# DomhnallBoyle/lip2speech-unit

Hardware: AMD Instinct MI355X
Metric: real-time factor (audio-sec/wall-sec), end-to-end lip->16kHz audio, 4s@25fps clips (higher is better)
Workload: dtype fp16

## Files before the change

include/lip2speech_hip.h:

```cpp
#ifndef LIP2SPEECH_HIP_H
#define LIP2SPEECH_HIP_H

#include <stddef.h>
#include <stdint.h>

#ifdef __cplusplus
extern "C" {
#endif

#define L2S_ABI_VERSION 16

enum { L2S_F16 = 0, L2S_BF16 = 1, L2S_F32 = 2 };

enum { L2S_OK = 0, L2S_EINVAL = -1, L2S_ESHAPE = -2, L2S_EALIGN = -3, L2S_EUNSUPPORTED = -4 };

enum {
  L2S_ACT_NONE = 0,
  L2S_ACT_RELU = 1,
  L2S_ACT_GELU = 2,
  L2S_ACT_SWISH = 3,
  L2S_ACT_PRELU = 4,
  L2S_ACT_LRELU = 5,
  L2S_ACT_TANH = 6
};

enum {
  L2S_F_RES_PRE  = 1 << 0,
  L2S_F_RES_POST = 1 << 1,
  L2S_F_ACCUM    = 1 << 2,
  L2S_F_DUAL     = 1 << 3,
  L2S_F_MASK     = 1 << 4,
  L2S_F_OUT_F32  = 1 << 5,
  L2S_F_RES_F32  = 1 << 6
};

enum {
  L2S_MODE_LINEAR = 0,
  L2S_MODE_CONV1D = 1,
  L2S_MODE_CONV2D = 2
};

typedef struct l2s_gemm_desc {
  const void* A;
  const void* W;
  void* C;
  void* C2;
  const float* bias;
  const float* slope;
  const void* R;
  const int32_t* lens;
  int32_t M, N, Cin, ntaps;
  int32_t lda, ldc, ldc2, ldr;
  int32_t mode;
  int32_t T_out, T_in, stride, dil, off;
  int32_t Ho, Wo, Hi, Wi, KW, pad;
  int32_t out_row_mul, out_row_add;
  int32_t mask_T, mask_mul;
  int32_t act, flags, dtype;
  float alpha;
  float act_slope;
  float slope2;
  int32_t groups, a_gstride, c_gstride;
  int64_t w_gstride;
  const int32_t* ktab;
} l2s_gemm_desc;
#define L2S_KTAB_MAX 9

int l2s_abi_version(void);
const char* l2s_build_info(void);

int l2s_tapgemm(const l2s_gemm_desc* host_desc, void* stream);
#define L2S_VARIANT_F32 2128128
int l2s_tapgemm_variant(const l2s_gemm_desc* host_desc);
#define L2S_EPI_FAMILY_F32 32
int l2s_tapgemm_epilogue_family(const l2s_gemm_desc* host_desc);

int l2s_stem_conv3d(const void* x, int x_is_f32, const void* w, const float* bias, const float* slope,
                    void* y, int B, int T, int H, int W, int dtype, void* stream);

int l2s_stem_pool_fused(const void* x, int x_is_f32, const void* w, const float* bias, const float* slope,
                        void* y, int B, int T, int H, int W, int dtype, void* stream);

int l2s_stem_pool_fused_u8(const uint8_t* frames, int Hin, int Win, int crop, float mean, float std, const void* w,
                           const float* bias, const float* slope, void* y, int B, int T, int dtype, void* stream);

int l2s_maxpool2d_3x3s2(const void* x, void* y, int N, int H, int W, int C, int dtype, void* stream);

int l2s_avgpool_hw(const void* x, void* y, int N, int HW, int C, int dtype, void* stream);

int l2s_layernorm(const void* x, int x_is_f32, int ldx, const float* gamma, const float* beta, float eps,
                  void* y, int y_is_f32, int ldy, void* y2, int ldy2, int M, int C, int zero_prefix,
                  const int32_t* lens, int len_mul, int mask_T, int dtype, void* stream);

int l2s_attention(const void* qkv, int ldq, void* out, int ldo, const void* pos, int ldp,
                  const float* bias_u, const float* bias_v, const int32_t* lens, int len_mul,
                  int B, int T, int H, int dtype, void* stream);

int l2s_glu_dwconv_swish(const void* x, const float* w, const float* bias, void* y, const int32_t* lens,
                         int len_mul, int B, int T, int C, int k, int dtype, void* stream);

int l2s_greedy_decode(const float* logits, int ldl, const int32_t* lens, int len_mul, int B, int T2, int V,
                      float temperature, float lenpen, int32_t* tokens, float* lprobs, float* score, void* stream);

int l2s_beam_decode(const float* logits, int ldl, const int32_t* lens, int len_mul, int B, int T2, int V, float temperature,
                    float lenpen, int beam, void* workspace, size_t workspace_bytes, int32_t* tokens, float* pos_scores,
                    float* score, int32_t* nhyp, void* stream);
size_t l2s_beam_decode_workspace(int B, int T2, int beam);

int l2s_ctc_frames(const float* logits, int ldl, const int32_t* lens, int len_mul, int B, int L, int V, int K, int32_t* labels,
                   int32_t* topk_cls, float* topk_lp, void* stream);

int l2s_ctc_beam_search(const int32_t* topk_cls, const float* topk_lp, const int32_t* lens, int len_mul, int B, int L, int K,
                        int beam, int nbest, void* workspace, size_t workspace_bytes, int32_t* labels, int32_t* lengths,
                        float* scores, void* stream);
size_t l2s_ctc_beam_workspace(int B, int L, int beam);
int l2s_ctc_repeat_labels(const int32_t* x, int ldx, const int32_t* lens, int len_mul, int B, int L, int32_t* y, int ldy,
                          void* stream);

int l2s_repeat2_cast(const float* x, void* y, int B, int T, int C, int dtype, void* stream);

int l2s_splitk_reduce(const float* P, int ldp, int S, float* x, int ldx, int M, int N, void* stream);

int l2s_splitk_reduce_layernorm(const float* P, int ldp, int S, float* x, int ldx, const float* gamma, const float* beta, float eps,
                                void* y, int y_is_f32, int ldy, int M, int C, const int32_t* lens, int len_mul, int mask_T,
                                int dtype, void* stream);

int l2s_cast_f32_to_16(const float* x, int ldx, void* y, int ldy, int M, int C, int dtype, void* stream);
int l2s_cast_16_to_f32(const void* x, int ldx, float* y, int ldy, int M, int C, int dtype, void* stream);
int l2s_broadcast_rows(const void* v, int ldv, void* y, int ldy, int col0, const int32_t* lens, int len_mul,
                       int B, int T, int C, int v_is_f32, int dtype, void* stream);
int l2s_transpose_ct_to_tc(const float* x, void* y, int ldy, int col0, const int32_t* lens, int len_mul,
                           int B, int C, int T, int dtype, void* stream);
int l2s_embedding(const int32_t* code, const void* table, void* y, int ldy, const int32_t* lens,
                  int B, int L, int C, int dtype, void* stream);
int l2s_embedding_tokens(const int32_t* tok, int ldt, int token_offset, const void* table, int n_rows, void* y, int ldy,
                         const int32_t* lens, int len_mul, int B, int L, int C, int dtype, void* stream);
int l2s_rows_f32_to_16_masked(const float* x, int ldx, void* y, int ldy, int col0, const int32_t* lens, int len_mul,
                              int B, int T, int C, int dtype, void* stream);
int l2s_lens_from_mask(const uint8_t* mask, int32_t* lens, int B, int T, void* stream);
int l2s_split_hi_lo(const float* x, int ldx, void* hi, void* lo, int ld16, int act, float slope, const int32_t* lens,
                    int len_mul, int B, int T, int C, int dtype, void* stream);

typedef struct l2s_respair_desc {
  const void* X; const void* W1; const void* W2; const float* b1; const float* b2;
  void* Y; float* XS; const int32_t* lens;
  int32_t len_mul, B, T, C, k, dil, last, accumulate, dtype;
  float slope;
} l2s_respair_desc;
int l2s_respair(const l2s_respair_desc* d, void* stream);

typedef struct l2s_respair_final_desc {
  const void* X[3]; const void* W1[3]; const void* W2[3]; const float* b1[3]; const float* b2[3];
  int32_t k[3], dil[3];
  void* Y; const int32_t* lens;
  int32_t n, len_mul, B, T, C, dtype;
  float slope;
} l2s_respair_final_desc;
int l2s_respair_final(const l2s_respair_final_desc* d, void* stream);

int l2s_basicblock_fused(const void* x, const void* w1, const float* b1, const float* s1, const void* w2, const float* b2,
                         const float* s2, void* y, int n_images, int H, int W, int C, int dtype, void* stream);
int l2s_basiclayer_fused(const void* x, const void* const* w, const float* const* bias, const float* const* slope, int n_blocks,
                         void* y, int n_images, int H, int W, int C, int dtype, void* stream);
int l2s_basicstage128_tail_fused(const void* x0, const void* t0, const void* wa, const float* ba, const float* sa, const void* w1,
                                 const float* b1, const float* s1, const void* w2, const float* b2, const float* s2, void* y,
                                 int n_images, int H, int W, int dtype, void* stream);

int l2s_conv_post_tanh(const float* x, const float* w, float bias, float* wav, int16_t* pcm, const int32_t* lens,
                       int len_mul, int B, int T, int C, int k, void* stream);

int l2s_resblock_fused(const void* xl, const void* w, const float* bias, float* xs, void* xl_out,
                       const int32_t* lens, int len_mul, int B, int T, int C, int k, int d0, int d1, int d2,
                       int accumulate, float slope, int dtype, void* stream);

int l2s_resstage_fused(const void* xl, const void* const* w, const float* const* bias, const int* ks, const int* dils,
                       int n_blocks, float* xs, void* xl_out, const int32_t* lens, int len_mul, int B, int T, int C,
                       float slope, int xs_final, int dtype, void* stream);

int l2s_preprocess_frames(const uint8_t* frames, void* y, int B, int T, int Hin, int Win, int crop, float mean,
                          float std, int dtype, void* stream);

int l2s_mel_spectrogram(const void* wav, int wav_is_i16, int64_t ldw, const int32_t* n_samples, int B, int S, const float* basis,
                        const float* fb, const int32_t* fb_range, float* mel, int ldm, int T_rows, int n_fft, int hop,
// ... 43 lines not shown
```

lip2speech_unit_amd/_lib.py:

```python
import ctypes
import os

_HERE = os.path.dirname(os.path.abspath(__file__))
LIB_PATH = os.environ.get("L2S_LIB_PATH") or os.path.join(_HERE, "liblip2speech_hip.so")

F16, BF16, F32 = 0, 1, 2
ACT_NONE, ACT_RELU, ACT_GELU, ACT_SWISH, ACT_PRELU, ACT_LRELU, ACT_TANH = range(7)
F_RES_PRE, F_RES_POST, F_ACCUM, F_DUAL, F_MASK, F_OUT_F32, F_RES_F32 = (1 << i for i in range(7))
MODE_LINEAR, MODE_CONV1D, MODE_CONV2D = 0, 1, 2
ABI_VERSION = 16

_ERR = {-1: "L2S_EINVAL", -2: "L2S_ESHAPE", -3: "L2S_EALIGN", -4: "L2S_EUNSUPPORTED"}


class L2SError(RuntimeError):
    pass


class GemmDesc(ctypes.Structure):
    _fields_ = [
        ("A", ctypes.c_void_p), ("W", ctypes.c_void_p), ("C", ctypes.c_void_p), ("C2", ctypes.c_void_p),
        ("bias", ctypes.c_void_p), ("slope", ctypes.c_void_p), ("R", ctypes.c_void_p), ("lens", ctypes.c_void_p),
        ("M", ctypes.c_int32), ("N", ctypes.c_int32), ("Cin", ctypes.c_int32), ("ntaps", ctypes.c_int32),
        ("lda", ctypes.c_int32), ("ldc", ctypes.c_int32), ("ldc2", ctypes.c_int32), ("ldr", ctypes.c_int32),
        ("mode", ctypes.c_int32),
        ("T_out", ctypes.c_int32), ("T_in", ctypes.c_int32), ("stride", ctypes.c_int32), ("dil", ctypes.c_int32),
        ("off", ctypes.c_int32),
        ("Ho", ctypes.c_int32), ("Wo", ctypes.c_int32), ("Hi", ctypes.c_int32), ("Wi", ctypes.c_int32),
        ("KW", ctypes.c_int32), ("pad", ctypes.c_int32),
        ("out_row_mul", ctypes.c_int32), ("out_row_add", ctypes.c_int32),
        ("mask_T", ctypes.c_int32), ("mask_mul", ctypes.c_int32),
        ("act", ctypes.c_int32), ("flags", ctypes.c_int32), ("dtype", ctypes.c_int32),
        ("alpha", ctypes.c_float), ("act_slope", ctypes.c_float), ("slope2", ctypes.c_float),
        ("groups", ctypes.c_int32), ("a_gstride", ctypes.c_int32), ("c_gstride", ctypes.c_int32),
        ("w_gstride", ctypes.c_int64),
        ("ktab", ctypes.c_void_p),
    ]


_vp, _i, _f = ctypes.c_void_p, ctypes.c_int, ctypes.c_float


class RespairDesc(ctypes.Structure):
    _fields_ = [("X", ctypes.c_void_p), ("W1", ctypes.c_void_p), ("W2", ctypes.c_void_p), ("b1", ctypes.c_void_p),
                ("b2", ctypes.c_void_p), ("Y", ctypes.c_void_p), ("XS", ctypes.c_void_p), ("lens", ctypes.c_void_p),
                ("len_mul", ctypes.c_int32), ("B", ctypes.c_int32), ("T", ctypes.c_int32), ("C", ctypes.c_int32),
                ("k", ctypes.c_int32), ("dil", ctypes.c_int32), ("last", ctypes.c_int32), ("accumulate", ctypes.c_int32),
                ("dtype", ctypes.c_int32), ("slope", ctypes.c_float)]


class RespairFinalDesc(ctypes.Structure):
    _fields_ = [("X", ctypes.c_void_p * 3), ("W1", ctypes.c_void_p * 3), ("W2", ctypes.c_void_p * 3), ("b1", ctypes.c_void_p * 3),
                ("b2", ctypes.c_void_p * 3), ("k", ctypes.c_int32 * 3), ("dil", ctypes.c_int32 * 3),
                ("Y", ctypes.c_void_p), ("lens", ctypes.c_void_p),
                ("n", ctypes.c_int32), ("len_mul", ctypes.c_int32), ("B", ctypes.c_int32), ("T", ctypes.c_int32),
                ("C", ctypes.c_int32), ("dtype", ctypes.c_int32), ("slope", ctypes.c_float)]


SIGNATURES = {
    "l2s_abi_version": ([], ctypes.c_int),
    "l2s_build_info": ([], ctypes.c_char_p),
    "l2s_tapgemm": ([ctypes.POINTER(GemmDesc), _vp], _i),
    "l2s_tapgemm_variant": ([ctypes.POINTER(GemmDesc)], _i),
    "l2s_tapgemm_epilogue_family": ([ctypes.POINTER(GemmDesc)], _i),
    "l2s_stem_conv3d": ([_vp, _i, _vp, _vp, _vp, _vp, _i, _i, _i, _i, _i, _vp], _i),
    "l2s_stem_pool_fused": ([_vp, _i, _vp, _vp, _vp, _vp, _i, _i, _i, _i, _i, _vp], _i),
    "l2s_stem_pool_fused_u8": ([_vp, _i, _i, _i, _f, _f, _vp, _vp, _vp, _vp, _i, _i, _i, _vp], _i),
    "l2s_maxpool2d_3x3s2": ([_vp, _vp, _i, _i, _i, _i, _i, _vp], _i),
    "l2s_avgpool_hw": ([_vp, _vp, _i, _i, _i, _i, _vp], _i),
    "l2s_layernorm": ([_vp, _i, _i, _vp, _vp, _f, _vp, _i, _i, _vp, _i, _i, _i, _i, _vp, _i, _i, _i, _vp], _i),
    "l2s_attention": ([_vp, _i, _vp, _i, _vp, _i, _vp, _vp, _vp, _i, _i, _i, _i, _i, _vp], _i),
    "l2s_glu_dwconv_swish": ([_vp, _vp, _vp, _vp, _vp, _i, _i, _i, _i, _i, _i, _vp], _i),
    "l2s_greedy_decode": ([_vp, _i, _vp, _i, _i, _i, _i, _f, _f, _vp, _vp, _vp, _vp], _i),
    "l2s_beam_decode": ([_vp, _i, _vp, _i, _i, _i, _i, _f, _f, _i, _vp, ctypes.c_size_t, _vp, _vp, _vp, _vp, _vp], _i),
    "l2s_beam_decode_workspace": ([_i, _i, _i], ctypes.c_size_t),
    "l2s_ctc_frames": ([_vp, _i, _vp, _i, _i, _i, _i, _i, _vp, _vp, _vp, _vp], _i),
    "l2s_ctc_beam_search": ([_vp, _vp, _vp, _i, _i, _i, _i, _i, _i, _vp, ctypes.c_size_t, _vp, _vp, _vp, _vp], _i),
    "l2s_ctc_beam_workspace": ([_i, _i, _i], ctypes.c_size_t),
    "l2s_ctc_repeat_labels": ([_vp, _i, _vp, _i, _i, _i, _vp, _i, _vp], _i),
    "l2s_repeat2_cast": ([_vp, _vp, _i, _i, _i, _i, _vp], _i),
    "l2s_splitk_reduce": ([_vp, _i, _i, _vp, _i, _i, _i, _vp], _i),
    "l2s_splitk_reduce_layernorm": ([_vp, _i, _i, _vp, _i, _vp, _vp, _f, _vp, _i, _i, _i, _i, _vp, _i, _i, _i, _vp], _i),
    "l2s_cast_f32_to_16": ([_vp, _i, _vp, _i, _i, _i, _i, _vp], _i),
    "l2s_cast_16_to_f32": ([_vp, _i, _vp, _i, _i, _i, _i, _vp], _i),
    "l2s_broadcast_rows": ([_vp, _i, _vp, _i, _i, _vp, _i, _i, _i, _i, _i, _i, _vp], _i),
    "l2s_transpose_ct_to_tc": ([_vp, _vp, _i, _i, _vp, _i, _i, _i, _i, _i, _vp], _i),
    "l2s_embedding": ([_vp, _vp, _vp, _i, _vp, _i, _i, _i, _i, _vp], _i),
    "l2s_embedding_tokens": ([_vp, _i, _i, _vp, _i, _vp, _i, _vp, _i, _i, _i, _i, _i, _vp], _i),
    "l2s_rows_f32_to_16_masked": ([_vp, _i, _vp, _i, _i, _vp, _i, _i, _i, _i, _i, _vp], _i),
    "l2s_lens_from_mask": ([_vp, _vp, _i, _i, _vp], _i),
    "l2s_basicblock_fused": ([_vp, _vp, _vp, _vp, _vp, _vp, _vp, _vp, _i, _i, _i, _i, _i, _vp], _i),
    "l2s_basiclayer_fused": ([_vp, _vp, _vp, _vp, _i, _vp, _i, _i, _i, _i, _i, _vp], _i),
    "l2s_basicstage128_tail_fused": ([_vp] * 12 + [_i, _i, _i, _i, _vp], _i),
    "l2s_split_hi_lo": ([_vp, _i, _vp, _vp, _i, _i, _f, _vp, _i, _i, _i, _i, _i, _vp], _i),
    "l2s_conv_post_tanh": ([_vp, _vp, _f, _vp, _vp, _vp, _i, _i, _i, _i, _i, _vp], _i),
    "l2s_resblock_fused": ([_vp, _vp, _vp, _vp, _vp, _vp, _i, _i, _i, _i, _i, _i, _i, _i, _i, _f, _i, _vp], _i),
    "l2s_resstage_fused": ([_vp, _vp, _vp, _vp, _vp, _i, _vp, _vp, _vp, _i, _i, _i, _i, _f, _i, _i, _vp], _i),
    "l2s_respair": ([ctypes.POINTER(RespairDesc), _vp], _i),
    "l2s_respair_final": ([ctypes.POINTER(RespairFinalDesc), _vp], _i),
    "l2s_preprocess_frames": ([_vp, _vp, _i, _i, _i, _i, _i, _f, _f, _i, _vp], _i),
    "l2s_mel_spectrogram": ([_vp, _i, ctypes.c_int64, _vp, _i, _i, _vp, _vp, _vp, _vp, _i, _i, _i, _i, _i, _f, _vp], _i),
    "l2s_stft_mel": ([_vp, _i, ctypes.c_int64, _vp, _i, _i, _vp, _vp, _vp, _vp, _i, _i, _i, _i, _i, _i, _f, _f, _vp], _i),
    "l2s_unit_ce": ([_vp, _i, _vp, _i, _vp, _i, _i, _i, _i, _i, _i, _vp, _vp, _vp, _vp, _vp], _i),
    "l2s_mel_l1_sc": ([_vp, _i, _vp, _i, _vp, _i, _i, _i, _i, _vp, _vp, _vp, _vp, _vp], _i),
    "l2s_ctc_loss_workspace": ([_i, _i, _i], ctypes.c_size_t),
    "l2s_ctc_loss": ([_vp, _i, _vp, _i, _i, _i, _i, _i, _vp, _vp, _vp, _i, _vp, ctypes.c_size_t, _vp, _vp], _i),
    "l2s_wave_stem_workspace": ([_i, _i], ctypes.c_size_t),
    "l2s_wave_stem": ([_vp, _i, ctypes.c_int64, _vp, _i, _i, _vp, _vp, _vp, _f, _vp, _i, _i, _i, _vp, ctypes.c_size_t, _i, _vp], _i),
    "l2s_kmeans_assign": ([_vp, _i, _vp, _vp, _vp, _i, _i, _i, _i, _i, _vp, _vp, _vp], _i),
    "l2s_kmeans_nearest_workspace": ([_i], ctypes.c_size_t),
    "l2s_kmeans_nearest": ([_vp, _i, ctypes.c_int64, _vp, _i, _vp, _vp, _i, _i, _vp, _vp, _vp, _vp, ctypes.c_size_t, _vp], _i),
    "l2s_kmeans_update_workspace": ([_i, _i], ctypes.c_size_t),
    "l2s_kmeans_update": ([_vp, _i, ctypes.c_int64, _vp, _i, _vp, _vp, _vp, _i, _i, _vp, _vp, _vp, _vp, ctypes.c_size_t, _vp], _i),
    "l2s_kmeans_pp_workspace": ([_i], ctypes.c_size_t),
    "l2s_kmeans_pp_pot": ([_vp, _i, ctypes.c_int64, _vp, _i, _i, _vp, _i, _vp, _vp, _vp, _vp, _vp, _vp, ctypes.c_size_t, _vp], _i),
    "l2s_kmeans_pp_pick": ([_vp, _i, _vp, _i, _vp, _vp, _vp, _vp], _i),
}

_lib = None


def load():
    global _lib
    if _lib is not None:
        return _lib
    if not os.path.exists(LIB_PATH):
        raise L2SError(
            f"{LIB_PATH} not found: build it with `python -c 'import __graft_entry__ as g; g.build()'` "
            "(make -C lip2speech_unit_amd/csrc). The MI355X path has no CPU fallback.")
    import torch
    lib = ctypes.CDLL(LIB_PATH)
    for name, (argtypes, restype) in SIGNATURES.items():
        try:
            fn = getattr(lib, name)
        except AttributeError as e:
            raise L2SError(f"{LIB_PATH} does not export {name}; rebuild the library") from e
        fn.argtypes = argtypes
        fn.restype = restype
    v = lib.l2s_abi_version()
    if v != ABI_VERSION:
        raise L2SError(f"ABI mismatch: library {v}, binding {ABI_VERSION}")
    _lib = lib
    return lib


def check(rc, what):
    if rc == 0:
        return
    if rc < 0:
        raise L2SError(f"{what}: rejected with {_ERR.get(rc, rc)}")
    raise L2SError(f"{what}: HIP launch failed with hipError_t={rc}")
```

lip2speech_unit_amd/conformer.py:

```python
import math
import os
from dataclasses import dataclass, field

import torch
import torch.nn as nn

from . import ops
from .ops import ACT_GELU, ACT_RELU, F_MASK, F_RES_POST, MODE_CONV1D


@dataclass
class ConformerConfig:
    conformer_embed_dim: int = 512
    conformer_attention_heads: int = 8
    conformer_ffn_embed_dim: int = 2048
    conformer_layers: int = 12
    cnn_module_kernel: int = 31
    encoder_embed_dim: int = 1024
    decoder_embed_dim: int = 204
    spk_dim: int = 256
    mel_dim: int = 160
    text_supervision: bool = field(default_factory=lambda: bool(int(os.environ.get("TEXT_SUPERVISION", 0))))
    text_classes: int = 4000

    @classmethod
    def from_model_cfg(cls, cfg):
        from .plugin import cfg_get
        c = cls()
        for k in ("conformer_embed_dim", "conformer_attention_heads", "conformer_ffn_embed_dim", "conformer_layers"):
            setattr(c, k, int(cfg_get(cfg, k, getattr(c, k))))
        c.text_supervision = bool(cfg_get(cfg, "text_supervision", c.text_supervision))
        return c


class TextClassifier(nn.Module):

    def __init__(self, d, num_classes):
        super().__init__()
        self.classifier = nn.Linear(d, num_classes)

    def _load_from_state_dict(self, state_dict, prefix, *a, **k):
        w = state_dict.get(prefix + "classifier.weight")
        if w is not None and w.dim() == 2 and w.shape[0] != self.classifier.out_features and w.shape[1] == self.classifier.in_features:
            self.classifier = nn.Linear(w.shape[1], w.shape[0])
        super()._load_from_state_dict(state_dict, prefix, *a, **k)


class PositionwiseFeedForward(nn.Module):
    def __init__(self, d, hidden):
        super().__init__()
        self.w_1 = nn.Linear(d, hidden)
        self.w_2 = nn.Linear(hidden, d)


class RelPositionMultiHeadedAttention(nn.Module):
    def __init__(self, heads, d):
        super().__init__()
        self.h, self.d_k = heads, d // heads
        self.linear_q = nn.Linear(d, d)
        self.linear_k = nn.Linear(d, d)
        self.linear_v = nn.Linear(d, d)
        self.linear_out = nn.Linear(d, d)
        self.linear_pos = nn.Linear(d, d, bias=False)
        self.pos_bias_u = nn.Parameter(torch.zeros(heads, d // heads))
        self.pos_bias_v = nn.Parameter(torch.zeros(heads, d // heads))


class ConvolutionModule(nn.Module):
    def __init__(self, ch, k):
        super().__init__()
        self.pointwise_cov1 = nn.Conv1d(ch, 2 * ch, 1)
        self.depthwise_conv = nn.Conv1d(ch, ch, k, padding=(k - 1) // 2, groups=ch)
        self.norm = nn.BatchNorm1d(ch)
        self.pointwise_cov2 = nn.Conv1d(ch, ch, 1)


class EncoderLayer(nn.Module):
    def __init__(self, d, heads, hidden, k):
        super().__init__()
        self.self_attn = RelPositionMultiHeadedAttention(heads, d)
        self.feed_forward = PositionwiseFeedForward(d, hidden)
        self.conv_module = ConvolutionModule(d, k)
        self.norm_ff = nn.LayerNorm(d, eps=1e-12)
        self.norm_mha = nn.LayerNorm(d, eps=1e-12)
        self.feed_forward_macaron = PositionwiseFeedForward(d, hidden)
        self.norm_ff_macaron = nn.LayerNorm(d, eps=1e-12)
        self.norm_conv = nn.LayerNorm(d, eps=1e-12)
        self.norm_final = nn.LayerNorm(d, eps=1e-12)


class RavenEncoderLayer(nn.Module):

    def __init__(self, d, heads, hidden):
        super().__init__()
        self.self_attn = RelPositionMultiHeadedAttention(heads, d)
        self.feed_forward = PositionwiseFeedForward(d, hidden)
        self.norm_ff = nn.BatchNorm1d(d)
        self.norm_mha = nn.LayerNorm(d, eps=1e-12)
        self.gamma_ff = nn.Parameter(0.1 * torch.ones(d))
        self.gamma_mha = nn.Parameter(0.1 * torch.ones(d))


class Encoder(nn.Module):

    def __init__(self, d, heads, hidden, blocks, k, idim=512, raven=False):
        super().__init__()
        self.frontend = None
        self.raven = raven
        self.embed = nn.Sequential(nn.Linear(idim, d))
        self.encoders = nn.ModuleList([RavenEncoderLayer(d, heads, hidden) if raven else EncoderLayer(d, heads, hidden, k)
                                       for _ in range(blocks)])
        self.after_norm = nn.LayerNorm(d, eps=1e-12)
        self.d, self.heads, self.hidden, self.k = d, heads, hidden, k
        self._packed = None
        self._pos_cache = {}
        if d // heads != 64:
            raise NotImplementedError("the attention kernels are built for 64-dim heads (512/8, 768/12, 1024/16)")

    def pack(self, dev, dtype):
        t16 = ops.torch_dtype(dtype)
        d = self.d
        inv = 1.0 / math.sqrt(d // self.heads)

        def w16(t):
            return t.detach().float().to(dev, t16).contiguous()

        P = {"layers": [], "dtype": dtype}
        P["w_emb"], P["b_emb"] = w16(self.embed[0].weight), _f32(self.embed[0].bias, dev)
        pos_w = []
        for L in self.encoders if self.raven else ():
            a, bn = L.self_attn, L.norm_ff
            g_m, g_f = L.gamma_mha.detach().float(), L.gamma_ff.detach().float()
            sc = bn.weight.detach().float() / torch.sqrt(bn.running_var.detach().float() + bn.eps)
            sh = bn.bias.detach().float() - bn.running_mean.detach().float() * sc
            w1 = L.feed_forward.w_1.weight.detach().float()
            e = {
                "ff": (w16(w1 * sc[None, :]), (w1 @ sh + L.feed_forward.w_1.bias.detach().float()).to(dev).contiguous(),
                       w16(L.feed_forward.w_2.weight.detach().float() * g_f[:, None]),
                       (L.feed_forward.w_2.bias.detach().float() * g_f).to(dev).contiguous()),
                "wqkv": w16(torch.cat([a.linear_q.weight.detach().float() * inv, a.linear_k.weight.detach().float(),
                                       a.linear_v.weight.detach().float()], 0)),
                "bqkv": torch.cat([a.linear_q.bias.detach().float() * inv, a.linear_k.bias.detach().float(),
                                   a.linear_v.bias.detach().float()], 0).to(dev).contiguous(),
                "u": (a.pos_bias_u.detach().float() * inv).to(dev).contiguous(),
                "v": (a.pos_bias_v.detach().float() * inv).to(dev).contiguous(),
                "wo": w16(a.linear_out.weight.detach().float() * g_m[:, None]),
                "bo": (a.linear_out.bias.detach().float() * g_m).to(dev).contiguous(),
                "n_mha": _ln(L.norm_mha, dev),
            }
            pos_w.append(a.linear_pos.weight.detach().float())
            P["layers"].append(e)
        for L in () if self.raven else self.encoders:
            a, c = L.self_attn, L.conv_module
            bn = c.norm
            sc = bn.weight.detach().float() / torch.sqrt(bn.running_var.detach().float() + bn.eps)
            sh = bn.bias.detach().float() - bn.running_mean.detach().float() * sc
            dw = c.depthwise_conv.weight.detach().float()[:, 0, :] * sc[:, None]
            db = c.depthwise_conv.bias.detach().float() * sc + sh
            e = {
                "ffm": (w16(L.feed_forward_macaron.w_1.weight), _f32(L.feed_forward_macaron.w_1.bias, dev),
                        w16(L.feed_forward_macaron.w_2.weight), _f32(L.feed_forward_macaron.w_2.bias, dev)),
                "ff": (w16(L.feed_forward.w_1.weight), _f32(L.feed_forward.w_1.bias, dev),
                       w16(L.feed_forward.w_2.weight), _f32(L.feed_forward.w_2.bias, dev)),
                "wqkv": w16(torch.cat([a.linear_q.weight.detach().float() * inv, a.linear_k.weight.detach().float(),
                                       a.linear_v.weight.detach().float()], 0)),
                "bqkv": torch.cat([a.linear_q.bias.detach().float() * inv, a.linear_k.bias.detach().float(),
                                   a.linear_v.bias.detach().float()], 0).to(dev).contiguous(),
                "u": (a.pos_bias_u.detach().float() * inv).to(dev).contiguous(),
                "v": (a.pos_bias_v.detach().float() * inv).to(dev).contiguous(),
                "wo": w16(a.linear_out.weight), "bo": _f32(a.linear_out.bias, dev),
                "pw1": w16(c.pointwise_cov1.weight[:, :, 0]), "pb1": _f32(c.pointwise_cov1.bias, dev),
                "dw": dw.t().contiguous().to(dev), "db": db.to(dev).contiguous(),
                "pw2": w16(c.pointwise_cov2.weight[:, :, 0]), "pb2": _f32(c.pointwise_cov2.bias, dev),
                "n_ffm": _ln(L.norm_ff_macaron, dev), "n_mha": _ln(L.norm_mha, dev), "n_conv": _ln(L.norm_conv, dev),
                "n_ff": _ln(L.norm_ff, dev), "n_fin": _ln(L.norm_final, dev),
            }
            pos_w.append(a.linear_pos.weight.detach().float())
            P["layers"].append(e)
        P["w_pos"] = w16(torch.cat(pos_w, 0))
        P["n_after"] = _ln(self.after_norm, dev)
        self._packed = P
        self._pos_cache = {}
        return P

    def _pos_proj(self, T, dev):
        key = (T, str(dev))
        if key not in self._pos_cache:
            P, d = self._packed, self.d
            dt = P["dtype"]
            t16 = ops.torch_dtype(dt)
            pe = rel_pos_table(T, d, dev).to(t16).contiguous()
            nl = len(P["layers"])
            out = torch.empty(2 * T - 1, nl * d, device=dev, dtype=t16)
            ops.tapgemm(pe, P["w_pos"], out, M=2 * T - 1, N=nl * d, Cin=d, dtype=dt)
            self._pos_cache[key] = out
        return self._pos_cache[key]

    def forward_rows(self, xin, lens, B, T, len_mul, dtype):
        dev = xin.device
        if self._packed is None or self._packed["b_emb"].device != dev or self._packed["dtype"] != dtype:
            self.pack(dev, dtype)
        P, dt = self._packed, dtype
        t16 = ops.torch_dtype(dt)
        d, H, F, k = self.d, self.heads, self.hidden, self.k
        M = B * T
        nl = len(P["layers"])
        x = torch.empty(M, d, device=dev, dtype=torch.float32)
        ops.tapgemm(xin, P["w_emb"], x, M=M, N=d, Cin=xin.shape[1], bias=P["b_emb"], alpha=math.sqrt(d), dtype=dt)
        pos = self._pos_proj(T, dev)
        h = torch.empty(M, d, device=dev, dtype=t16)
        f = torch.empty(M, F, device=dev, dtype=t16)
        qkv = torch.empty(M, 3 * d, device=dev, dtype=t16)
        att = torch.empty(M, d, device=dev, dtype=t16)
        glu_in = torch.empty(M, 2 * d, device=dev, dtype=t16)
        cv = torch.empty(M, d, device=dev, dtype=t16)

        def half_ffn(e, name, norm, after, y):
            w = e[name]
            ops.layernorm(x, norm[0], norm[1], 1e-12, h, M=M, C=d, dtype=dt)
            ops.tapgemm(h, w[0], f, M=M, N=F, Cin=d, bias=w[1], act=ACT_RELU, dtype=dt)
            ops.residual_linear(f, w[2], w[3], x, M=M, N=d, K=F, alpha=0.5, dtype=dt, cache=e, key=name,
                                ln=(after[0], after[1], 1e-12, y))

        for li, e in enumerate(P["layers"] if self.raven else ()):
            ops.layernorm(x, e["n_mha"][0], e["n_mha"][1], 1e-12, h, M=M, C=d, dtype=dt)
            ops.tapgemm(h, e["wqkv"], qkv, M=M, N=3 * d, Cin=d, bias=e["bqkv"], dtype=dt)
            ops.attention(qkv, att, B=B, T=T, H=H, pos=pos[:, li * d:], ldp=nl * d, bias_u=e["u"], bias_v=e["v"],
                          lens=lens, len_mul=len_mul, dtype=dt)
            ops.tapgemm(att, e["wo"], x, M=M, N=d, Cin=d, bias=e["bo"], R=x, ldr=d, flags=F_RES_POST, dtype=dt)
            ops.cast_f32_to_16(x, h, M, d, dt)
            w = e["ff"]
            ops.tapgemm(h, w[0], f, M=M, N=F, Cin=d, bias=w[1], act=ACT_RELU, dtype=dt)
            ops.tapgemm(f, w[2], x, M=M, N=d, Cin=F, bias=w[3], R=x, ldr=d, flags=F_RES_POST, dtype=dt)
        for li, e in enumerate(() if self.raven else P["layers"]):
            half_ffn(e, "ffm", e["n_ffm"], e["n_mha"], h)
            ops.tapgemm(h, e["wqkv"], qkv, M=M, N=3 * d, Cin=d, bias=e["bqkv"], dtype=dt)
            ops.attention(qkv, att, B=B, T=T, H=H, pos=pos[:, li * d:], ldp=nl * d, bias_u=e["u"], bias_v=e["v"],
                          lens=lens, len_mul=len_mul, dtype=dt)
            ops.tapgemm(att, e["wo"], x, M=M, N=d, Cin=d, bias=e["bo"], R=x, ldr=d, flags=F_RES_POST, dtype=dt)
            ops.layernorm(x, e["n_conv"][0], e["n_conv"][1], 1e-12, h, M=M, C=d, dtype=dt)
            ops.tapgemm(h, e["pw1"], glu_in, M=M, N=2 * d, Cin=d, bias=e["pb1"], dtype=dt)
            ops.glu_dwconv_swish(glu_in, e["dw"], e["db"], cv, B=B, T=T, C=d, k=k, lens=lens, len_mul=len_mul, dtype=dt)
            ops.tapgemm(cv, e["pw2"], x, M=M, N=d, Cin=d, bias=e["pb2"], R=x, ldr=d, flags=F_RES_POST, dtype=dt)
            half_ffn(e, "ff", e["n_ff"], e["n_fin"], x)
        return x


def _f32(t, dev):
    return t.detach().float().to(dev).contiguous()


def _ln(m, dev):
    return (_f32(m.weight, dev), _f32(m.bias, dev))


def rel_pos_table(T, d, dev):
    rel = torch.arange(T - 1, -T, -1, dtype=torch.float32).unsqueeze(1)
    div = torch.exp(torch.arange(0, d, 2, dtype=torch.float32) * -(math.log(10000.0) / d))
    pe = torch.zeros(2 * T - 1, d)
    pe[:, 0::2] = torch.sin(rel * div)
    pe[:, 1::2] = torch.cos(rel * div)
    return pe.to(dev)


class Conformer(nn.Module):

    def __init__(self, cfg: ConformerConfig = None, dtype=ops.F16):
        super().__init__()
        cfg = cfg or ConformerConfig()
        self.cfg = cfg
        d = cfg.conformer_embed_dim
        self.encoder = Encoder(d, cfg.conformer_attention_heads, cfg.conformer_ffn_embed_dim, cfg.conformer_layers,
                               cfg.cnn_module_kernel)
        self.proj_in = nn.Linear(cfg.encoder_embed_dim, d) if cfg.encoder_embed_dim != d else None
        self.proj_out = nn.Linear(d, cfg.decoder_embed_dim) if cfg.decoder_embed_dim != d else None
        self.mel_conv = nn.Sequential(
            nn.Conv1d(d + cfg.spk_dim, d, 3, 1, 1), nn.Dropout(0.0), nn.GELU(),
            nn.Conv1d(d, d, 3, 1, 1), nn.Dropout(0.0), nn.GELU(),
            nn.Conv1d(d, d, 3, 1, 1), nn.Dropout(0.0), nn.GELU())
        self.mel_proj = nn.Linear(d, cfg.mel_dim)
        self.text_classifier = TextClassifier(d, cfg.text_classes) if cfg.text_supervision else None
        self.dtype = dtype
        self._packed = None

    @property
    def _pos_cache(self):
        return self.encoder._pos_cache

    @_pos_cache.setter
    def _pos_cache(self, v):
        self.encoder._pos_cache = v

    def load_state_dict(self, *a, **k):
        r = super().load_state_dict(*a, **k)
        self._packed = None
        self.encoder._packed, self.encoder._pos_cache = None, {}
        return r

    def pack(self, dev):
        t16 = ops.torch_dtype(self.dtype)
        cfg = self.cfg

        def w16(t):
            return t.detach().float().to(dev, t16).contiguous()

        P = {}
        if self.proj_in is not None:
            P["w_in"], P["b_in"] = w16(self.proj_in.weight), _f32(self.proj_in.bias, dev)
        self.encoder.pack(dev, self.dtype)
        P["n_after"] = self.encoder._packed["n_after"]
        P["mel"] = []
        for i in (0, 3, 6):
            cv = self.mel_conv[i]
            P["mel"].append((w16(cv.weight.detach().permute(0, 2, 1).reshape(cv.weight.shape[0], -1)),
                             _f32(cv.bias, dev), cv.weight.shape[1]))
        D = cfg.mel_dim
        perm = torch.tensor([2 * k + j for j in range(2) for k in range(D // 2)])
        P["w_mel"], P["b_mel"] = w16(self.mel_proj.weight.detach()[perm]), _f32(self.mel_proj.bias.detach()[perm], dev)
        if self.proj_out is not None:
            P["w_out"], P["b_out"] = w16(self.proj_out.weight), _f32(self.proj_out.bias, dev)
        if self.text_classifier is not None:
            lin = self.text_classifier.classifier
            V = lin.out_features
            Vp = -(-V // 4) * 4
            w = torch.zeros(Vp, lin.in_features)
# ... 95 lines not shown
```

lip2speech_unit_amd/csrc/conformer_conv.hip:

```cpp
#include "l2s_common.h"

namespace {

constexpr int CT = 64, KMAX = 31;

template <typename ET, int TT>
__global__ __launch_bounds__(256) void glu_dwconv_kernel(const uint16_t* __restrict__ x, const float* __restrict__ w,
                                                         const float* __restrict__ bias, uint16_t* __restrict__ y,
                                                         const int32_t* __restrict__ lens, int len_mul, int T, int C,
                                                         int k) {
  constexpr int OPT = TT / 4;
  __shared__ float g[(TT + KMAX - 1) * CT];
  const int b = blockIdx.z, t0 = blockIdx.x * TT, c0 = blockIdx.y * CT;
  const int half = (k - 1) / 2, rows = TT + k - 1;
  int lim = lens ? lens[b] * len_mul : T;
  lim = lim < T ? lim : T;
  for (int i = threadIdx.x; i < rows * (CT / 8); i += 256) {
    const int r = i / (CT / 8), ch = i - r * (CT / 8);
    const int t = t0 + r - half;
    float o[8] = {0.f, 0.f, 0.f, 0.f, 0.f, 0.f, 0.f, 0.f};
    if (t >= 0 && t < lim) {
      const uint16_t* rp = x + ((int64_t)b * T + t) * (2 * C) + c0 + ch * 8;
      frag16 a, gt;
      a.u = *reinterpret_cast<const uint4*>(rp);
      gt.u = *reinterpret_cast<const uint4*>(rp + C);
#pragma unroll
      for (int e = 0; e < 8; ++e) o[e] = ET::to_f32(a.s[e]) * __builtin_amdgcn_rcpf(1.0f + __expf(-ET::to_f32(gt.s[e])));
    }
#pragma unroll
    for (int e = 0; e < 8; ++e) g[r * CT + ch * 8 + e] = o[e];
  }
  __syncthreads();
  const int c = threadIdx.x & 63, tq = threadIdx.x >> 6;
  float wr[KMAX];
#pragma unroll
  for (int j = 0; j < KMAX; ++j) wr[j] = j < k ? w[j * C + c0 + c] : 0.f;
  const float bs = bias[c0 + c];
  float win[OPT + KMAX - 1];
#pragma unroll
  for (int j = 0; j < OPT + KMAX - 1; ++j) win[j] = (tq * OPT + j < rows) ? g[(tq * OPT + j) * CT + c] : 0.f;
#pragma unroll
  for (int o = 0; o < OPT; ++o) {
    const int t = t0 + tq * OPT + o;
    float acc = bs;
#pragma unroll
    for (int j = 0; j < KMAX; ++j) acc += win[o + j] * wr[j];
    acc = l2s_swish(acc);
    if (t < T) y[((int64_t)b * T + t) * C + c0 + c] = ET::from_f32(t < lim ? acc : 0.f);
  }
}

}

int l2s_f32_glu_dwconv_swish(const void* x, const float* w, const float* bias, void* y, const int32_t* lens, int len_mul, int B, int T,
                             int C, int k, hipStream_t st);

extern "C" int l2s_glu_dwconv_swish(const void* x, const float* w, const float* bias, void* y, const int32_t* lens,
                                    int len_mul, int B, int T, int C, int k, int dtype, void* stream) {
  if (!x || !w || !bias || !y) return L2S_EINVAL;
  if (B <= 0 || T <= 0 || C <= 0) return L2S_ESHAPE;
  if (k <= 0 || k > KMAX || !(k & 1)) return L2S_EUNSUPPORTED;
  if (C % CT) return L2S_EALIGN;
  if (dtype == L2S_F32) return l2s_f32_glu_dwconv_swish(x, w, bias, y, lens, len_mul, B, T, C, k, (hipStream_t)stream);
  const int r128 = ((T + 127) / 128) * 128, r100 = ((T + 99) / 100) * 100;
  const bool use100 = r100 + ((T + 99) / 100) * 10 < r128 + ((T + 127) / 128) * 10;
  const int TTr = use100 ? 100 : 128;
  dim3 grid((T + TTr - 1) / TTr, C / CT, B), blk(256);
  hipStream_t st = (hipStream_t)stream;
#define GLU_LAUNCH(ET_, TT_) hipLaunchKernelGGL((glu_dwconv_kernel<ET_, TT_>), grid, blk, 0, st, (const uint16_t*)x, w, bias, (uint16_t*)y, lens, len_mul, T, C, k)
  if (dtype == L2S_F16) { if (use100) GLU_LAUNCH(ElemF16, 100); else GLU_LAUNCH(ElemF16, 128); }
  else if (dtype == L2S_BF16) { if (use100) GLU_LAUNCH(ElemBF16, 100); else GLU_LAUNCH(ElemBF16, 128); }
  else return L2S_EINVAL;
#undef GLU_LAUNCH
  L2S_CHECK_LAUNCH();
  return L2S_OK;
}
```

lip2speech_unit_amd/csrc/phasegemm.hip:

```cpp
#include "l2s_common.h"
#include "tapgemm_tiles.h"
#include <cstdlib>

int l2s_phasegemm_f16_m0(const l2s_gemm_desc& d, hipStream_t st);
int l2s_phasegemm_f16_m1(const l2s_gemm_desc& d, hipStream_t st);
int l2s_phasegemm_f16_m2(const l2s_gemm_desc& d, hipStream_t st);
int l2s_phasegemm_bf16_m0(const l2s_gemm_desc& d, hipStream_t st);
int l2s_phasegemm_bf16_m1(const l2s_gemm_desc& d, hipStream_t st);
int l2s_phasegemm_bf16_m2(const l2s_gemm_desc& d, hipStream_t st);
int l2s_phasegemm_f16_m3(const l2s_gemm_desc& d, hipStream_t st);
int l2s_phasegemm_bf16_m3(const l2s_gemm_desc& d, hipStream_t st);

int l2s_phasegemm_ktab_launch(const l2s_gemm_desc& d, hipStream_t st) {
  if (d.mode != L2S_MODE_LINEAR || d.groups < 1) return L2S_EINVAL;
  const int fam = l2s::pick_epilogue(d.flags, d.act);
  if (fam != 2 && fam != l2s::L2S_EPI_G16A) return L2S_EUNSUPPORTED;
  if ((d.Cin % 64) || d.N < 256 || d.M < 256 || (d.M & 7) || (d.N & 7) || (d.lda & 7) || (d.ldc & 7) || (d.c_gstride & 63) ||
      (d.ldr & 7) || d.out_row_mul != 1 || d.out_row_add != 0)
    return L2S_EUNSUPPORTED;
  return d.dtype == L2S_F16 ? l2s_phasegemm_f16_m3(d, st) : l2s_phasegemm_bf16_m3(d, st);
}

bool l2s_phasegemm_eligible(const l2s_gemm_desc& d) {
  static const int mode = [] { const char* e = getenv("L2S_PHASEGEMM"); return e ? atoi(e) : 1; }();
  if (mode == 0) return false;
  if (d.groups > 1 || d.mode < 0 || d.mode > 2 || d.ktab) return false;
  if (d.mode == L2S_MODE_LINEAR && d.ntaps != 1) return false;
  if (d.mode == L2S_MODE_CONV1D && (d.T_out <= 0 || d.T_in <= 0)) return false;
  if (d.mode == L2S_MODE_CONV2D && (d.Ho <= 0 || d.Wo <= 0 || d.KW <= 0 || d.ntaps % d.KW)) return false;
  const int fam = l2s::pick_epilogue(d.flags, d.act);
  if (fam == l2s::L2S_EPI_ALL && !(l2s::is_x32(d.flags, d.act) && !(d.ldc & 3) && !(d.ldr & 3) && !(d.ldc2 & 3))) return false;
  static const int res_on = [] { const char* e = getenv("L2S_PHASEGEMM_RES"); return e ? atoi(e) : 1; }();
  if (!res_on && (fam == l2s::L2S_EPI_G16A || fam == l2s::L2S_EPI_G16B)) return false;
  if (fam == l2s::L2S_EPI_S32 && ((d.ldc & 3) || (d.ldr & 3))) return false;
  if ((d.Cin % 64) || d.N < 256 || d.M < 256 || (d.lda & 7)) return false;
  if (d.mode == L2S_MODE_LINEAR && ((d.M & 7) || (d.N & 7))) return false;
  if (mode == 2) return true;
  auto cdivl = [](long a, long b) { return (a + b - 1) / b; };
  const long tm = cdivl(d.M, 256);
  const long rounds_big = cdivl(tm * cdivl(d.N, 256), 256);
  if (rounds_big * ((long)d.Cin * d.ntaps / 64) < 20) return false;
  const double big = (double)rounds_big * 2.0 / 1.2;
  const double reg = (double)cdivl(tm * cdivl(d.N, 128), 256);
  return big < reg;
}

#ifdef L2S_WITH_WIDEGEMM
int l2s_widegemm_f16(const l2s_gemm_desc& d, hipStream_t st);
int l2s_widegemm_bf16(const l2s_gemm_desc& d, hipStream_t st);
static bool wide_ok(const l2s_gemm_desc& d) {
  static const int mode = [] { const char* e = getenv("L2S_WIDEGEMM"); return e ? atoi(e) : 0; }();
  if (mode == 0 || d.mode != L2S_MODE_LINEAR) return false;
  const int fam = l2s::pick_epilogue(d.flags, d.act);
  if (fam > l2s::L2S_EPI_G16A && fam != l2s::L2S_EPI_S32) return false;
  return !(d.M & 7) && !(d.N & 7);
}
#endif

int l2s_phasegemm_launch(const l2s_gemm_desc& d, hipStream_t st) {
  const bool h = d.dtype == L2S_F16;
#ifdef L2S_WITH_WIDEGEMM
  if (wide_ok(d)) return h ? l2s_widegemm_f16(d, st) : l2s_widegemm_bf16(d, st);
#endif
  switch (d.mode) {
    case L2S_MODE_LINEAR: return h ? l2s_phasegemm_f16_m0(d, st) : l2s_phasegemm_bf16_m0(d, st);
    case L2S_MODE_CONV1D: return h ? l2s_phasegemm_f16_m1(d, st) : l2s_phasegemm_bf16_m1(d, st);
    case L2S_MODE_CONV2D: return h ? l2s_phasegemm_f16_m2(d, st) : l2s_phasegemm_bf16_m2(d, st);
    default: return L2S_EINVAL;
  }
}
```

lip2speech_unit_amd/csrc/phasegemm_kernel.h:

```cpp
#pragma once
#include "tapgemm_common.h"
#include <cstdlib>

using namespace l2s;

namespace {

constexpr int PBM = 256, PBN = 256, PBK = 64;
constexpr int Q_B = 128 * PBK * 2;
constexpr bool p_generic(int epi) { return epi == L2S_EPI_G16A || epi == L2S_EPI_G16B; }
constexpr int p_scr_b(int epi) { return p_generic(epi) ? 16 * 64 * 4 : 16 * (4 * 32 + 16); }
constexpr int p_smem(int epi) { return 8 * Q_B + 8 * p_scr_b(epi); }

#ifdef L2S_PHASE_STAMPS
__device__ unsigned long long* g_phase_stamps = nullptr;
#define PHSTAMP(i) { const unsigned long long now_ = __builtin_amdgcn_s_memtime(); ph_acc[i] += now_ - ph_last; ph_last = now_; }
#else
#define PHSTAMP(i)
#endif

constexpr int PG_KTAB = 3;
template <typename ET, int MODE_T, int EPI>
__global__ __launch_bounds__(512) void phasegemm_kernel(const l2s_gemm_desc p, const int tilesM, const int tilesN,
                                                        const int chunk, const int band) {
  constexpr bool KT = MODE_T == PG_KTAB;
  constexpr int MODE = KT ? (int)L2S_MODE_LINEAR : MODE_T;
  constexpr int MI = 8, NI = 4;
#ifdef L2S_NO_PAIRED
  constexpr bool PAIRED = false;
#else
  constexpr bool PAIRED = EPI <= L2S_EPI_G16A;
#endif
  extern __shared__ __attribute__((aligned(16))) uint16_t lds[];
  const int tid = threadIdx.x, lane = tid & 63;
  const int wave = __builtin_amdgcn_readfirstlane(tid >> 6);
  const int wr = wave >> 2, wc = wave & 3;
  const int K = p.Cin * p.ntaps;
  const int nk = K / PBK;
  const uint16_t* zero = reinterpret_cast<const uint16_t*>(&g_zero16);

  const int tiles_mn = tilesM * tilesN;
  const int ntiles = tiles_mn * (KT ? p.groups : 1);
  const int slot = blockIdx.x >> 3, slots = gridDim.x >> 3;
  const int lo = (blockIdx.x & 7) * chunk;
  const int hi = lo + chunk < ntiles ? lo + chunk : ntiles;
  const int my_n = (lo + slot < hi) ? (hi - lo - slot + slots - 1) / slots : 0;
  if (my_n == 0) return;
  const int total_q = my_n * nk * 4;
  auto tile_coords = [&](int i, int& m0, int& n0, int& g) {
    int l = lo + slot + i * slots;
    g = 0;
    if constexpr (KT) {
      const int per_m = p.groups * tilesN;
      const int mt = l / per_m, r = l - mt * per_m;
      g = r / tilesN;
      m0 = mt * PBM;
      n0 = (r - g * tilesN) * PBN;
      return;
    }
    const int bsz = band * tilesN;
    const int bi = l / bsz, idx = l - bi * bsz;
    const int rows = tilesM - bi * band < band ? tilesM - bi * band : band;
    const int tn = idx / rows;
    m0 = (bi * band + idx - tn * rows) * PBM;
    n0 = tn * PBN;
  };

  const int srow = lane >> 3;
  const int schunk = (lane & 7) ^ (srow & 7);
  const uint16_t* qa_ptr[2][2];
  int qa_t[2][2], qa_x[2][2];
  const uint16_t* qb_ptr[2][2];
  int run_tap = 0, run_c = 0, run_ky = 0, run_kx = 0;
  const char* sa_base[2][2] = {{nullptr, nullptr}, {nullptr, nullptr}};
  const char* sw_base[2][2] = {{nullptr, nullptr}, {nullptr, nullptr}};
  uint32_t a_lane = 0, w_lane[2] = {0, 0};
  if constexpr (MODE == L2S_MODE_LINEAR) {
    a_lane = (uint32_t)(srow * p.lda * 2 + (schunk << 4));
#pragma unroll
    for (int j = 0; j < 2; ++j) {
      const int within = 16 * (wave & 1) + 8 * j + srow;
      const int bchunk = PAIRED ? ((lane & 7) ^ paired_w_key(within)) : schunk;
      w_lane[j] = (uint32_t)(srow * K * 2 + (bchunk << 4));
    }
  }
  typedef const int32_t __attribute__((address_space(4)))* ktab_ptr_t;
  constexpr int KTN = L2S_KTAB_MAX;
  const ktab_ptr_t kt_tab = (ktab_ptr_t)(uintptr_t)p.ktab;
  ktab_ptr_t kt_row = kt_tab;
  int nk_stage = nk, kt_blk = 0, kt_win = 0;
  uint32_t kt_cur_a = 0, kt_cur_w = 0, kt_nxt_a = 0, kt_nxt_w = 0;
  const int kpb = KT ? p.Cin / PBK : 1;
  auto setup_issue = [&](int i) {
    int m0, n0, tg;
    tile_coords(i, m0, n0, tg);
    if constexpr (KT) {
      kt_row = kt_tab + tg * (2 + 2 * KTN);
      nk_stage = kt_row[0] * kpb;
      kt_blk = 0; kt_win = 0;
      kt_cur_a = (uint32_t)kt_row[2] * 2u; kt_cur_w = (uint32_t)kt_row[2 + KTN] * 2u;
      kt_nxt_a = (uint32_t)kt_row[3] * 2u; kt_nxt_w = (uint32_t)kt_row[3 + KTN] * 2u;
    }
#ifdef L2S_ABL_SAMETILE
    m0 = 0; n0 = 0;
#endif
    if constexpr (MODE == L2S_MODE_LINEAR) {
#pragma unroll
      for (int h = 0; h < 2; ++h)
#pragma unroll
        for (int j = 0; j < 2; ++j) {
          int mg = m0 + (wave >> 2) * 128 + h * 64 + 16 * (wave & 3) + 8 * j;
          mg = mg < p.M ? mg : p.M - 8;
          sa_base[h][j] = (const char*)p.A + (int64_t)mg * p.lda * 2;
          int ng = n0 + (wave >> 1) * 64 + h * 32 + 16 * (wave & 1) + 8 * j;
          ng = ng < p.N ? ng : p.N - 8;
          sw_base[h][j] = (const char*)p.W + (int64_t)ng * K * 2;
        }
      return;
    }
#pragma unroll
    for (int h = 0; h < 2; ++h)
#pragma unroll
      for (int j = 0; j < 2; ++j) {
        int m = m0 + (wave >> 2) * 128 + h * 64 + 16 * (wave & 3) + 8 * j + srow;
        m = m < p.M ? m : p.M - 1;
        qa_t[h][j] = 0; qa_x[h][j] = 0;
        if (MODE == L2S_MODE_LINEAR) {
          qa_ptr[h][j] = (const uint16_t*)p.A + (int64_t)m * p.lda + schunk * 8;
        } else if (MODE == L2S_MODE_CONV1D) {
          const int b = m / p.T_out, t = m - b * p.T_out;
          qa_ptr[h][j] = (const uint16_t*)p.A + (int64_t)b * p.T_in * p.lda + schunk * 8;
          qa_t[h][j] = t * p.stride + p.off;
        } else {
          const int hw = p.Ho * p.Wo;
          const int img = m / hw, rem = m - img * hw;
          const int oy = rem / p.Wo, ox = rem - oy * p.Wo;
          qa_ptr[h][j] = (const uint16_t*)p.A + (int64_t)img * p.Hi * p.Wi * p.lda + schunk * 8;
          qa_t[h][j] = oy * p.stride - p.pad;
          qa_x[h][j] = ox * p.stride - p.pad;
        }
        const int within = 16 * (wave & 1) + 8 * j + srow;
        int n = n0 + (wave >> 1) * 64 + h * 32 + within;
        n = n < p.N ? n : p.N - 1;
        const int bchunk = PAIRED ? ((lane & 7) ^ paired_w_key(within)) : schunk;
        qb_ptr[h][j] = (const uint16_t*)p.W + (int64_t)n * K + bchunk * 8;
      }
  };
  auto slot_off = [&](int b, int e) -> uint32_t { return (uint32_t)((b * 4 + e) * Q_B); };
  int s_i = 0, s_kt = 0, s_e = 0, s_par = 0, staged = 0;
  auto stage_one = [&](auto e_tag) {
    constexpr int E = decltype(e_tag)::value;
    const bool live = staged < total_q;
    const int k0 = s_kt * PBK;
    const int se = E >= 0 ? E : s_e;
    uint16_t* dst = lds + (slot_off(s_par, se) >> 1) + wave * 1024;
    const bool is_a = (se == 0) || (se == 3);
    const int h = (se == 2 || se == 3) ? 1 : 0;
    if constexpr (MODE == L2S_MODE_LINEAR) {
      static_assert(E >= 0, "LINEAR stages with a compile-time element");
      const uint32_t kb = (uint32_t)k0 * 2u;
      const uint32_t kba = KT ? kt_cur_a : kb, kbw = KT ? kt_cur_w : kb;
#pragma unroll
      for (int j = 0; j < 2; ++j) {
        const char* g = is_a ? sa_base[h][j] + (size_t)kba + (size_t)a_lane : sw_base[h][j] + (size_t)kbw + (size_t)w_lane[j];
#ifdef L2S_ABL_ZEROSRC
        g = (const char*)zero;
#endif
#if defined(L2S_ABL_WARMDMA)
        if (staged < 8) __builtin_amdgcn_global_load_lds((gptr_t)g, (lptr_t)(dst + j * 512), 16, 0, 0);
#elif !defined(L2S_ABL_NODMA)
        __builtin_amdgcn_global_load_lds((gptr_t)g, (lptr_t)(dst + j * 512), 16, 0, 0);
#endif
      }
      return;
    }
#pragma unroll
    for (int j = 0; j < 2; ++j) {
      const uint16_t* g;
      bool ok = live;
      if (!is_a) {
        g = qb_ptr[h][j] + k0;
      } else if (MODE == L2S_MODE_LINEAR) {
        g = qa_ptr[h][j] + k0;
      } else if (MODE == L2S_MODE_CONV1D) {
        const int st = qa_t[h][j] + run_tap * p.dil;
        ok = ok && ((unsigned)st < (unsigned)p.T_in);
        g = qa_ptr[h][j] + (st * p.lda + run_c);
      } else {
        const int iy = qa_t[h][j] + run_ky, ix = qa_x[h][j] + run_kx;
        ok = ok && ((unsigned)iy < (unsigned)p.Hi) && ((unsigned)ix < (unsigned)p.Wi);
        g = qa_ptr[h][j] + ((iy * p.Wi + ix) * p.lda + run_c);
      }
      g = ok ? g : zero;
#ifdef L2S_ABL_ZEROSRC
      g = zero;
#endif
#ifndef L2S_ABL_NODMA
// ... 94 lines not shown
    constexpr int Q = decltype(q_tag)::value;
#ifndef L2S_ABL_NOREAD
    if (Q == 0) { read_b(fb[0], lds_base + slot_off(par, 1)); __builtin_amdgcn_sched_barrier(0); read_a(lds_base + slot_off(par, 0)); }
    if (Q == 1) read_b(fb[1], lds_base + slot_off(par, 2));
    if (Q == 2) read_a(lds_base + slot_off(par, 3));
#endif
    stage_one(std::integral_constant<int, (Q + 2) & 3>{});
    __builtin_amdgcn_sched_barrier(0);
    wait_vmcnt<8>();
    asm volatile("" ::: "memory");
    __builtin_amdgcn_s_barrier();
    asm volatile("" ::: "memory");
    lds_wait();
    __builtin_amdgcn_s_setprio(1);
    constexpr int RH = (Q >= 2) ? 1 : 0, CH = (Q == 1 || Q == 2) ? 1 : 0;
#ifdef L2S_ABL_MFMA32
    {
      typedef __attribute__((ext_vector_type(16))) float f32x16_t;
#pragma unroll
      for (int mb = 0; mb < 2; ++mb) {
        f32x16_t c;
#pragma unroll
        for (int e = 0; e < 16; ++e) c[e] = acc[RH * 4 + mb * 2 + (e >> 3)][CH * 2 + ((e >> 2) & 1)][e & 3];
#pragma unroll
        for (int kk = 0; kk < 4; ++kk)
          c = __builtin_amdgcn_mfma_f32_32x32x16_f16(fb[CH][kk >> 1][kk & 1].h, fa[mb * 2 + (kk >> 1)][kk & 1].h, c, 0, 0, 0);
#pragma unroll
        for (int e = 0; e < 16; ++e) acc[RH * 4 + mb * 2 + (e >> 3)][CH * 2 + ((e >> 2) & 1)][e & 3] = c[e];
      }
    }
#elif !defined(L2S_ABL_NOMFMA)
#pragma unroll
    for (int i = 0; i < 4; ++i)
#pragma unroll
      for (int j = 0; j < 2; ++j) {
        acc[RH * 4 + i][CH * 2 + j] = ET::mfma(fb[CH][j][0], fa[i][0], acc[RH * 4 + i][CH * 2 + j]);
        acc[RH * 4 + i][CH * 2 + j] = ET::mfma(fb[CH][j][1], fa[i][1], acc[RH * 4 + i][CH * 2 + j]);
      }
#endif
    __builtin_amdgcn_s_setprio(0);
    __builtin_amdgcn_sched_barrier(0);
    asm volatile("" ::: "memory");
    __builtin_amdgcn_s_barrier();
    asm volatile("" ::: "memory");
    __builtin_amdgcn_sched_barrier(0);
    stage_advance();
  };

  int par = 0;
#ifdef L2S_PHASE_STAMPS
  unsigned long long ph_acc[4] = {0, 0, 0, 0};
  unsigned long long ph_last = __builtin_amdgcn_s_memtime();
  const unsigned long long ph_t0 = ph_last;
#endif
  auto nk_of = [&](int ti) -> int {
    if (ti >= my_n) return 0;
    const int l = lo + slot + ti * slots;
    const int per_m = p.groups * tilesN;
    return kt_tab[((l % per_m) / tilesN) * (2 + 2 * KTN)] * kpb;
  };
  int nk_next = KT ? nk_of(0) : nk;
  for (int ti = 0; ti < my_n; ++ti) {
    const int nk_c = nk_next;
    if constexpr (KT) nk_next = nk_of(ti + 1);
    for (int kt = 0; kt < nk_c; ++kt) {
#ifdef L2S_PHASE_STAMPS
      if (kt == 1) PHSTAMP(2)
#endif
      phase(std::integral_constant<int, 0>{}, par);
      phase(std::integral_constant<int, 1>{}, par);
      phase(std::integral_constant<int, 2>{}, par);
      phase(std::integral_constant<int, 3>{}, par);
      par ^= 1;
    }
    PHSTAMP(0)
    int m0, n0, grp;
    tile_coords(ti, m0, n0, grp);
    const uint32_t scr = lds_base + 8 * Q_B + (uint32_t)wave * p_scr_b(EPI);
    auto rowmap = [&](int m) -> int64_t { return m < p.M ? (int64_t)m * p.out_row_mul + p.out_row_add : (int64_t)-1; };
    if constexpr (EPI == L2S_EPI_X32) {
      epilogue_stream32x<ET, MI, NI>(p, acc, lane, m0 + wr * 128, n0 + wc * 64, rowmap);
    } else if constexpr (EPI == L2S_EPI_S32) {
      epilogue_direct32<ET, MI, NI>(p, acc, lane, m0 + wr * 128, n0 + wc * 64, grp, rowmap);
    } else if constexpr (PAIRED) {
      epilogue_direct16<ET, MI, NI, EPI, decltype(rowmap), NoHook, true>(p, acc, lane, m0 + wr * 128, n0 + wc * 64, grp, rowmap);
    } else if constexpr (EPI == L2S_EPI_G16A) {
      epilogue_impl<ET, MI, NI, F_G16A, true, true>(p, acc, scr, lane, m0 + wr * 128, n0 + wc * 64, grp, rowmap);
    } else if constexpr (EPI == L2S_EPI_G16B) {
      epilogue_impl<ET, MI, NI, F_G16B, true, true>(p, acc, scr, lane, m0 + wr * 128, n0 + wc * 64, grp, rowmap);
    } else {
      epilogue_fast16<ET, MI, NI, (EPI - L2S_EPI_F16) / 2, ((EPI - L2S_EPI_F16) & 1) != 0, 1>(
          p, acc, scr, lane, m0 + wr * 128, n0 + wc * 64, grp, rowmap);
    }
#pragma unroll
    for (int i = 0; i < MI; ++i)
#pragma unroll
      for (int j = 0; j < NI; ++j) acc[i][j] = f32x4_t{0.f, 0.f, 0.f, 0.f};
    PHSTAMP(1)
  }
  wait_vmcnt<0>();
#ifdef L2S_PHASE_STAMPS
  if (lane == 0 && (wave == 0 || wave == 7) && g_phase_stamps) {
    unsigned long long* o = g_phase_stamps + ((int64_t)blockIdx.x * 2 + (wave ? 1 : 0)) * 8;
    for (int i = 0; i < 3; ++i) o[i] = ph_acc[i];
    o[3] = (unsigned long long)my_n;
    o[4] = __builtin_amdgcn_s_memtime() - ph_t0;
    o[5] = (unsigned long long)nk;
  }
#endif
}

template <typename ET, int MODE, int EPI>
int launch_phase(const l2s_gemm_desc& d, hipStream_t st) {
  auto kern = phasegemm_kernel<ET, MODE, EPI>;
  static L2sSmemOptIn opt_in;
  if (int e = l2s_smem_opt_in(kern, p_smem(EPI), opt_in)) return e;
  const int tilesM = (d.M + PBM - 1) / PBM, tilesN = (d.N + PBN - 1) / PBN;
  const int ntiles = tilesM * tilesN * (MODE == PG_KTAB ? d.groups : 1);
  const int chunk = (ntiles + 7) / 8;
  const int slots = chunk < 32 ? chunk : 32;
  const double ap = (double)PBM * d.Cin * 2.0, wp = (double)PBN * d.Cin * d.ntaps * 2.0;
  auto cdivi = [](int a, int b) { return (a + b - 1) / b; };
  int band = 1;
  double best = 1e300;
  for (int b = 1; b <= tilesM; ++b) {
    const int wn = cdivi(chunk, b) < tilesN ? cdivi(chunk, b) : tilesN;
    const int an = b * cdivi(chunk, b * tilesN);
    const double fp = ap * (an < tilesM ? an : tilesM) + wp * wn;
    if (fp < best) { best = fp; band = b; }
  }
  hipLaunchKernelGGL(kern, dim3(8 * slots), dim3(512), p_smem(EPI), st, d, tilesM, tilesN, chunk, band);
  L2S_CHECK_LAUNCH();
  return L2S_OK;
}


#ifdef L2S_PHASE_STAMPS
int phase_set_stamps(void* buf) { return (int)hipMemcpyToSymbol(HIP_SYMBOL(g_phase_stamps), &buf, sizeof(buf)); }
#endif

template <typename ET, int MODE>
int launch_phase_mode(const l2s_gemm_desc& d, hipStream_t st) {
  if constexpr (MODE == PG_KTAB) {
    switch (pick_epilogue(d.flags, d.act)) {
      case 2: return launch_phase<ET, MODE, 2>(d, st);
      case L2S_EPI_G16A: return launch_phase<ET, MODE, L2S_EPI_G16A>(d, st);
      default: return L2S_EUNSUPPORTED;
    }
  } else {
    switch (pick_epilogue(d.flags, d.act)) {
      case 0: return launch_phase<ET, MODE, 0>(d, st);
      case 1: return launch_phase<ET, MODE, 1>(d, st);
      case 2: return launch_phase<ET, MODE, 2>(d, st);
      case 3: return launch_phase<ET, MODE, 3>(d, st);
      case 4: return launch_phase<ET, MODE, 4>(d, st);
      case 5: return launch_phase<ET, MODE, 5>(d, st);
      case L2S_EPI_G16A: return launch_phase<ET, MODE, L2S_EPI_G16A>(d, st);
      case L2S_EPI_G16B: return launch_phase<ET, MODE, L2S_EPI_G16B>(d, st);
      case L2S_EPI_S32: return launch_phase<ET, MODE, L2S_EPI_S32>(d, st);
      case L2S_EPI_ALL: return is_x32(d.flags, d.act) ? launch_phase<ET, MODE, L2S_EPI_X32>(d, st) : (int)L2S_EUNSUPPORTED;
      default: return L2S_EUNSUPPORTED;
    }
  }
}

}
```

lip2speech_unit_amd/csrc/tapgemm.hip:

```cpp
#include "l2s_common.h"
#include "tapgemm_tiles.h"

using l2s::pick_tile;

#define L2S_DECL(m, e)                                                     \
  int l2s_tapgemm_f16_m##m##_e##e(const l2s_gemm_desc& d, hipStream_t st); \
  int l2s_tapgemm_bf16_m##m##_e##e(const l2s_gemm_desc& d, hipStream_t st);
#define L2S_DECL_MODE(m) L2S_DECL(m, 0) L2S_DECL(m, 1) L2S_DECL(m, 2) L2S_DECL(m, 3) L2S_DECL(m, 4) L2S_DECL(m, 5) \
                         L2S_DECL(m, 6) L2S_DECL(m, 7) L2S_DECL(m, 8) L2S_DECL(m, 9)
L2S_DECL_MODE(0) L2S_DECL_MODE(1) L2S_DECL_MODE(2)
#undef L2S_DECL_MODE
#undef L2S_DECL

static int launch_dtype_mode(const l2s_gemm_desc& d, hipStream_t st) {
  typedef int (*fn_t)(const l2s_gemm_desc&, hipStream_t);
#define L2S_E(t, m, e) l2s_tapgemm_##t##_m##m##_e##e
#define L2S_ROW(t, m) {L2S_E(t, m, 0), L2S_E(t, m, 1), L2S_E(t, m, 2), L2S_E(t, m, 3), L2S_E(t, m, 4), \
                       L2S_E(t, m, 5), L2S_E(t, m, 6), L2S_E(t, m, 7), L2S_E(t, m, 8), L2S_E(t, m, 9)}
  static const fn_t table[2][3][l2s::L2S_EPI_COUNT] = {{L2S_ROW(f16, 0), L2S_ROW(f16, 1), L2S_ROW(f16, 2)},
                                                       {L2S_ROW(bf16, 0), L2S_ROW(bf16, 1), L2S_ROW(bf16, 2)}};
#undef L2S_ROW
#undef L2S_E
  if (d.mode < 0 || d.mode > 2) return L2S_EINVAL;
  return table[d.dtype == L2S_F16 ? 0 : 1][d.mode][l2s::pick_epilogue(d.flags, d.act)](d, st);
}

bool l2s_phasegemm_eligible(const l2s_gemm_desc& d);
int l2s_phasegemm_launch(const l2s_gemm_desc& d, hipStream_t st);
int l2s_phasegemm_ktab_launch(const l2s_gemm_desc& d, hipStream_t st);
bool l2s_patchconv_eligible(const l2s_gemm_desc& d);
int l2s_patchconv_launch(const l2s_gemm_desc& d, hipStream_t st);
int l2s_tapgemm_f32_launch(const l2s_gemm_desc& d, hipStream_t st);
static bool patch_enabled() {
  static const bool on = [] { const char* e = getenv("L2S_NO_PATCHCONV"); return !(e && atoi(e)); }();
  return on;
}

extern "C" int l2s_tapgemm(const l2s_gemm_desc* hd, void* stream) {
  if (!hd) return L2S_EINVAL;
  l2s_gemm_desc d = *hd;
  if (!d.A || !d.W || !d.C) return L2S_EINVAL;
  if (d.M <= 0 || d.N <= 0 || d.Cin <= 0 || d.ntaps <= 0) return L2S_ESHAPE;
  if (d.groups <= 0) d.groups = 1;
  if (d.out_row_mul <= 0) d.out_row_mul = 1;
  if (d.dtype == L2S_F32) {
    if (((uintptr_t)d.A & 15) || ((uintptr_t)d.W & 15) || ((uintptr_t)d.C & 3)) return L2S_EALIGN;
    if ((d.flags & (L2S_F_RES_PRE | L2S_F_RES_POST)) && !d.R) return L2S_EINVAL;
    if ((d.flags & L2S_F_DUAL) && !d.C2) return L2S_EINVAL;
    if ((d.flags & L2S_F_MASK) && (!d.lens || d.mask_T <= 0 || d.mask_mul <= 0)) return L2S_EINVAL;
    if (d.act == L2S_ACT_PRELU && !d.slope) return L2S_EINVAL;
    if (d.mode == L2S_MODE_CONV1D && (d.T_out <= 0 || d.T_in <= 0)) return L2S_ESHAPE;
    if (d.mode == L2S_MODE_CONV2D && (d.Ho <= 0 || d.Wo <= 0 || d.Hi <= 0 || d.Wi <= 0 || d.KW <= 0)) return L2S_ESHAPE;
    if ((int64_t)d.M * d.out_row_mul + d.out_row_add >= ((int64_t)1 << 31)) return L2S_EUNSUPPORTED;
    return l2s_tapgemm_f32_launch(d, (hipStream_t)stream);
  }
  if ((d.Cin & 7) || (d.lda & 7) || (d.N & 3) || (d.ldc & 3) || (d.a_gstride & 7) || (d.c_gstride & 3) ||
      (d.w_gstride & 7))
    return L2S_EALIGN;
  if (((uintptr_t)d.A & 15) || ((uintptr_t)d.W & 15) || ((uintptr_t)d.C & 15)) return L2S_EALIGN;
  if ((d.flags & (L2S_F_RES_PRE | L2S_F_RES_POST)) && (!d.R || (d.ldr & 3))) return L2S_EINVAL;
  if ((d.flags & L2S_F_DUAL) && (!d.C2 || (d.ldc2 & 3))) return L2S_EINVAL;
  if ((d.flags & L2S_F_MASK) && (!d.lens || d.mask_T <= 0 || d.mask_mul <= 0)) return L2S_EINVAL;
  if (d.act == L2S_ACT_PRELU && !d.slope) return L2S_EINVAL;
  if (d.mode == L2S_MODE_CONV1D && (d.T_out <= 0 || d.T_in <= 0)) return L2S_ESHAPE;
  if (d.mode == L2S_MODE_CONV2D && (d.Ho <= 0 || d.Wo <= 0 || d.Hi <= 0 || d.Wi <= 0 || d.KW <= 0)) return L2S_ESHAPE;
  if (d.mode != L2S_MODE_LINEAR && (int64_t)d.Cin * d.ntaps > (1 << 15)) return L2S_EUNSUPPORTED;
  if ((int64_t)d.M * d.out_row_mul + d.out_row_add >= ((int64_t)1 << 31)) return L2S_EUNSUPPORTED;
  hipStream_t st = (hipStream_t)stream;
  if (d.dtype != L2S_F16 && d.dtype != L2S_BF16) return L2S_EINVAL;
  if (d.ktab) return l2s_phasegemm_ktab_launch(d, st);
  if (l2s_phasegemm_eligible(d)) return l2s_phasegemm_launch(d, st);
  if (patch_enabled() && l2s_patchconv_eligible(d)) return l2s_patchconv_launch(d, st);
  return launch_dtype_mode(d, st);
}

extern "C" int l2s_tapgemm_variant(const l2s_gemm_desc* hd) {
  if (!hd || hd->M <= 0 || hd->N <= 0) return L2S_EINVAL;
  if (hd->dtype == L2S_F32) return hd->ktab ? L2S_EUNSUPPORTED : L2S_VARIANT_F32;
  if (hd->ktab || l2s_phasegemm_eligible(*hd)) return 256256;
  if (patch_enabled() && l2s_patchconv_eligible(*hd)) return 999000 + hd->N;
  return pick_tile(hd->M, hd->N, hd->groups > 0 ? hd->groups : 1);
}

extern "C" int l2s_tapgemm_epilogue_family(const l2s_gemm_desc* hd) {
  if (!hd) return L2S_EINVAL;
  if (hd->dtype == L2S_F32) return L2S_EPI_FAMILY_F32;
  return l2s::pick_epilogue(hd->flags, hd->act);
}
```

lip2speech_unit_amd/csrc/tapgemm_common.h:

```cpp
#pragma once
#include "l2s_common.h"
#include "tapgemm_tiles.h"
#include <type_traits>

namespace l2s {

typedef __attribute__((address_space(1))) const void* gptr_t;
typedef __attribute__((address_space(3))) void* lptr_t;

__device__ const uint4 g_zero16 = {0u, 0u, 0u, 0u};

typedef unsigned u32x4_t __attribute__((ext_vector_type(4)));

template <int OFF>
__device__ __forceinline__ void lds_read_b128(frag16& f, uint32_t addr) {
  u32x4_t v;
  asm volatile("ds_read_b128 %0, %1 offset:%2" : "=v"(v) : "v"(addr), "n"(OFF));
  f.u = make_uint4(v.x, v.y, v.z, v.w);
}
__device__ __forceinline__ void lds_wait() {
  __builtin_amdgcn_sched_barrier(0);
  asm volatile("s_waitcnt lgkmcnt(0)" ::: "memory");
  __builtin_amdgcn_sched_barrier(0);
}
template <int N>
__device__ __forceinline__ void lds_wait_n() {
  __builtin_amdgcn_sched_barrier(0);
  asm volatile("s_waitcnt lgkmcnt(%0)" ::"n"(N) : "memory");
  __builtin_amdgcn_sched_barrier(0);
}

template <int OFF>
__device__ __forceinline__ void lds_write_f4(uint32_t addr, f32x4_t v) {
  asm volatile("ds_write_b128 %0, %1 offset:%2" ::"v"(addr), "v"(v), "n"(OFF) : "memory");
}
template <int OFF>
__device__ __forceinline__ f32x4_t lds_read_f4(uint32_t addr) {
  f32x4_t v;
  asm volatile("ds_read_b128 %0, %1 offset:%2" : "=v"(v) : "v"(addr), "n"(OFF));
  return v;
}

typedef unsigned u32x2_t __attribute__((ext_vector_type(2)));
template <int OFF>
__device__ __forceinline__ void lds_write_b64(uint32_t addr, u32x2_t v) {
  asm volatile("ds_write_b64 %0, %1 offset:%2" ::"v"(addr), "v"(v), "n"(OFF) : "memory");
}
__device__ __forceinline__ void lds_write_b64_at(uint32_t addr, u32x2_t v, const int off) {
  asm volatile("ds_write_b64 %0, %1 offset:%2" ::"v"(addr), "v"(v), "n"(off) : "memory");
}
__device__ __forceinline__ u32x4_t lds_read_u4(uint32_t addr) {
  u32x4_t v;
  asm volatile("ds_read_b128 %0, %1" : "=v"(v) : "v"(addr));
  return v;
}

template <int N>
__device__ __forceinline__ void wait_vmcnt() {
  asm volatile("s_waitcnt vmcnt(%0)" ::"n"(N) : "memory");
}


template <int MI, int NI>
__host__ __device__ constexpr int epilogue_scratch_bytes() {
  constexpr int a = 16 * (NI * 16 + 4) * 4, b = (MI >= 2 ? 32 : 16) * (NI * 32 + 16);
  return a > b ? a : b;
}

constexpr int F_G16A = L2S_F_RES_PRE | L2S_F_RES_POST;
constexpr int F_G16B = L2S_F_RES_PRE | L2S_F_RES_POST | L2S_F_DUAL | L2S_F_MASK;
constexpr int F_S32 = L2S_F_RES_PRE | L2S_F_RES_POST | L2S_F_OUT_F32 | L2S_F_RES_F32;

template <typename ET, int MI, int NI, int FEAT, bool LIN, bool SWZ = false, typename RowMap>
__device__ __forceinline__ void epilogue_impl(const l2s_gemm_desc& p, f32x4_t (&acc)[MI][NI], const uint32_t scr,
                                              const int lane, const int row_base, const int ncol_base, const int grp,
                                              RowMap rowmap) {
  constexpr int WAVE_N = NI * 16;
  constexpr int LPR = WAVE_N / 8;
  constexpr int SROW = SWZ ? WAVE_N : WAVE_N + 4;
  static_assert(!SWZ || NI == 4, "swizzled scratch: 16 chunks of 16 B per row");
  const int lm = lane & 15, lg = lane >> 4;
  const uint32_t scr_w = scr + (uint32_t)(lm * SROW + lg * 4) * 4;
  const int rr = lane / LPR, cc = lane - rr * LPR;
  const uint32_t scr_r = scr + (uint32_t)(rr * SROW + cc * 8) * 4;
  constexpr int RPP_ = 64 / LPR, PASSES_ = RPP_ < 16 ? 16 / RPP_ : 1;
  uint32_t swz_w[NI], swz_lo[PASSES_], swz_hi[PASSES_];
  (void)swz_w; (void)swz_lo; (void)swz_hi; (void)scr_w; (void)scr_r;
  if constexpr (SWZ) {
#pragma unroll
    for (int j = 0; j < NI; ++j)
      swz_w[j] = scr + (uint32_t)(lm * 256 + (((j ^ (lm >> 2)) << 6) | ((lg ^ (lm & 3)) << 4)));
#pragma unroll
    for (int h = 0; h < PASSES_; ++h) {
      const int r = rr + h * RPP_;
      swz_lo[h] = scr + (uint32_t)(r * 256 + (((2 * cc) ^ r) << 4));
      swz_hi[h] = scr + (uint32_t)(r * 256 + (((2 * cc + 1) ^ r) << 4));
    }
  }
  const bool lane_on = lane < 16 * LPR;
  const int flags = p.flags & FEAT;
  const int n = ncol_base + cc * 8;
  const bool ok_lo = lane_on && (n < p.N), ok_hi = lane_on && (n + 4 < p.N);
  const int col = grp * p.c_gstride + n;
  const float* bias = p.bias ? p.bias + grp * p.N : nullptr;
  const float* slope = (p.act == L2S_ACT_PRELU) ? p.slope + grp * p.N : nullptr;
  float bv[8], sv[8];
#pragma unroll
  for (int e = 0; e < 8; ++e) { bv[e] = 0.f; sv[e] = 0.f; }
  if (bias && ok_lo) { const float4 q = *reinterpret_cast<const float4*>(bias + n); bv[0] = q.x; bv[1] = q.y; bv[2] = q.z; bv[3] = q.w; }
  if (bias && ok_hi) { const float4 q = *reinterpret_cast<const float4*>(bias + n + 4); bv[4] = q.x; bv[5] = q.y; bv[6] = q.z; bv[7] = q.w; }
  if (slope && ok_lo) { const float4 q = *reinterpret_cast<const float4*>(slope + n); sv[0] = q.x; sv[1] = q.y; sv[2] = q.z; sv[3] = q.w; }
  if (slope && ok_hi) { const float4 q = *reinterpret_cast<const float4*>(slope + n + 4); sv[4] = q.x; sv[5] = q.y; sv[6] = q.z; sv[7] = q.w; }
  float sl[8];
  {
    const float s_uni = p.act == L2S_ACT_RELU ? 0.f : (p.act == L2S_ACT_LRELU ? p.act_slope : 1.f);
#pragma unroll
    for (int e = 0; e < 8; ++e) sl[e] = p.act == L2S_ACT_PRELU ? sv[e] : s_uni;
  }
  const bool has_res = (flags & (L2S_F_RES_PRE | L2S_F_RES_POST)) != 0;
  auto ld8 = [&](const void* base, int64_t row, int ld, bool f32, float(&out)[8]) {
    if (f32) {
      const float* q = (const float*)base + row * ld + col;
      if (ok_lo) { const float4 t = *reinterpret_cast<const float4*>(q); out[0] = t.x; out[1] = t.y; out[2] = t.z; out[3] = t.w; }
      if (ok_hi) { const float4 t = *reinterpret_cast<const float4*>(q + 4); out[4] = t.x; out[5] = t.y; out[6] = t.z; out[7] = t.w; }
    } else {
      const uint16_t* q = (const uint16_t*)base + row * ld + col;
      if (ok_lo) {
        const uint2 t = *reinterpret_cast<const uint2*>(q);
        out[0] = ET::to_f32((uint16_t)(t.x & 0xffff)); out[1] = ET::to_f32((uint16_t)(t.x >> 16));
        out[2] = ET::to_f32((uint16_t)(t.y & 0xffff)); out[3] = ET::to_f32((uint16_t)(t.y >> 16));
      }
      if (ok_hi) {
        const uint2 t = *reinterpret_cast<const uint2*>(q + 4);
        out[4] = ET::to_f32((uint16_t)(t.x & 0xffff)); out[5] = ET::to_f32((uint16_t)(t.x >> 16));
        out[6] = ET::to_f32((uint16_t)(t.y & 0xffff)); out[7] = ET::to_f32((uint16_t)(t.y >> 16));
      }
    }
  };
  const bool st16_uniform = ((p.N & 7) == 0) && ((p.c_gstride & 7) == 0 || grp == 0) && ((ncol_base & 7) == 0);
  auto st8_16 = [&](void* base, int64_t row, int ld, const float(&v)[8]) {
    uint16_t* q = (uint16_t*)base + row * ld + col;
    uint4 t;
    t.x = ET::pack2(v[0], v[1]);
    t.y = ET::pack2(v[2], v[3]);
    t.z = ET::pack2(v[4], v[5]);
    t.w = ET::pack2(v[6], v[7]);
    if (st16_uniform && (((uintptr_t)base & 15) == 0) && ((ld & 7) == 0)) {
      *reinterpret_cast<uint4*>(q) = t;
    } else if (ok_hi && (((uintptr_t)q & 15) == 0)) {
      *reinterpret_cast<uint4*>(q) = t;
    } else {
      if (ok_lo) *reinterpret_cast<uint2*>(q) = make_uint2(t.x, t.y);
      if (ok_hi) *reinterpret_cast<uint2*>(q + 4) = make_uint2(t.z, t.w);
    }
  };
  constexpr int RPP = 64 / LPR, PASSES = RPP < 16 ? 16 / RPP : 1;
// ... 3 lines not shown
  constexpr int c0 = decltype(c0_tag)::value;
  int orow[CH][PASSES];
  uint4 rraw[CH][PASSES][2];
  int mt[CH][PASSES], mlen[CH][PASSES];
#pragma unroll
  for (int i = c0; i < c0 + CH; ++i)
#pragma unroll
    for (int h = 0; h < PASSES; ++h) {
      const int o = (int)rowmap(row_base + i * 16 + rr + h * RPP);
      orow[i - c0][h] = (lane_on && ok_lo) ? o : -1;
      mt[i - c0][h] = 0;
      mlen[i - c0][h] = 1;
      if ((flags & L2S_F_MASK) && orow[i - c0][h] >= 0) {
        const int clip = (int)((unsigned)o / (unsigned)p.mask_T);
        mt[i - c0][h] = o - clip * p.mask_T;
        mlen[i - c0][h] = p.lens[clip];
      }
      rraw[i - c0][h][0] = make_uint4(0, 0, 0, 0);
      rraw[i - c0][h][1] = make_uint4(0, 0, 0, 0);
      if (has_res && orow[i - c0][h] >= 0) {
        if (flags & L2S_F_RES_F32) {
          const float* q = (const float*)p.R + (int64_t)o * p.ldr + col;
          rraw[i - c0][h][0] = *reinterpret_cast<const uint4*>(q);
          if (ok_hi) rraw[i - c0][h][1] = *reinterpret_cast<const uint4*>(q + 4);
        } else {
          const uint16_t* q = (const uint16_t*)p.R + (int64_t)o * p.ldr + col;
          const uint2 a = *reinterpret_cast<const uint2*>(q);
          const uint2 b = ok_hi ? *reinterpret_cast<const uint2*>(q + 4) : make_uint2(0, 0);
          rraw[i - c0][h][0] = make_uint4(a.x, a.y, b.x, b.y);
        }
      }
    }
#pragma unroll
  for (int i = c0; i < c0 + CH; ++i) {
    f32x4_t lo_[PASSES], hi_[PASSES];
    if constexpr (SWZ) {
#pragma unroll
      for (int j = 0; j < NI; ++j) lds_write_f4<0>(swz_w[j], acc[i][j]);
      asm volatile("s_waitcnt lgkmcnt(0)" ::: "memory");
#pragma unroll
      for (int h = 0; h < PASSES; ++h) { lo_[h] = lds_read_f4<0>(swz_lo[h]); hi_[h] = lds_read_f4<0>(swz_hi[h]); }
    } else {
    lds_write_f4<0>(scr_w, acc[i][0]);
    if (NI > 1) lds_write_f4<64>(scr_w, acc[i][NI > 1 ? 1 : 0]);
    if (NI > 2) lds_write_f4<128>(scr_w, acc[i][NI > 2 ? 2 : 0]);
    if (NI > 3) lds_write_f4<192>(scr_w, acc[i][NI > 3 ? 3 : 0]);
    asm volatile("s_waitcnt lgkmcnt(0)" ::: "memory");
    lo_[0] = lds_read_f4<0>(scr_r);
    hi_[0] = lds_read_f4<16>(scr_r);
    if (PASSES > 1) {
      lo_[PASSES - 1] = lds_read_f4<RPP * SROW * 4>(scr_r);
      hi_[PASSES - 1] = lds_read_f4<RPP * SROW * 4 + 16>(scr_r);
    }
    }
    lds_wait();
#pragma unroll
    for (int h = 0; h < PASSES; ++h) {
    const f32x4_t lo = lo_[h], hi = hi_[h];
    const int64_t o = orow[i - c0][h];
    if (o < 0) continue;
    const bool keep = !(flags & L2S_F_MASK) || (mt[i - c0][h] < mlen[i - c0][h] * p.mask_mul);
    float rv[8] = {0.f, 0.f, 0.f, 0.f, 0.f, 0.f, 0.f, 0.f}, cv[8] = {0.f, 0.f, 0.f, 0.f, 0.f, 0.f, 0.f, 0.f};
    if (has_res) {
      const uint4 r0 = rraw[i - c0][h][0], r1 = rraw[i - c0][h][1];
      if (flags & L2S_F_RES_F32) {
        rv[0] = __builtin_bit_cast(float, r0.x); rv[1] = __builtin_bit_cast(float, r0.y);
        rv[2] = __builtin_bit_cast(float, r0.z); rv[3] = __builtin_bit_cast(float, r0.w);
        rv[4] = __builtin_bit_cast(float, r1.x); rv[5] = __builtin_bit_cast(float, r1.y);
        rv[6] = __builtin_bit_cast(float, r1.z); rv[7] = __builtin_bit_cast(float, r1.w);
      } else {
        rv[0] = ET::to_f32((uint16_t)(r0.x & 0xffff)); rv[1] = ET::to_f32((uint16_t)(r0.x >> 16));
        rv[2] = ET::to_f32((uint16_t)(r0.y & 0xffff)); rv[3] = ET::to_f32((uint16_t)(r0.y >> 16));
        rv[4] = ET::to_f32((uint16_t)(r0.z & 0xffff)); rv[5] = ET::to_f32((uint16_t)(r0.z >> 16));
        rv[6] = ET::to_f32((uint16_t)(r0.w & 0xffff)); rv[7] = ET::to_f32((uint16_t)(r0.w >> 16));
      }
    }
    if (flags & L2S_F_ACCUM) ld8(p.C, o, p.ldc, (flags & L2S_F_OUT_F32) != 0, cv);
    float v[8] = {lo[0], lo[1], lo[2], lo[3], hi[0], hi[1], hi[2], hi[3]};
#pragma unroll
    for (int e = 0; e < 8; ++e) v[e] = v[e] + bv[e];
    if (p.alpha != 1.f) {
#pragma unroll
      for (int e = 0; e < 8; ++e) v[e] *= p.alpha;
    }
    if (flags & L2S_F_RES_PRE) {
#pragma unroll
      for (int e = 0; e < 8; ++e) v[e] += rv[e];
    }
    if (LIN) {
      if (p.act != L2S_ACT_NONE) {
#pragma unroll
        for (int e = 0; e < 8; ++e) v[e] = fmaxf(v[e], 0.f) + fminf(v[e], 0.f) * sl[e];
      }
    } else {
    switch (p.act) {
      case L2S_ACT_RELU:
#pragma unroll
        for (int e = 0; e < 8; ++e) v[e] = fmaxf(v[e], 0.f);
        break;
      case L2S_ACT_GELU:
#pragma unroll
        for (int e = 0; e < 8; ++e) v[e] = l2s_gelu(v[e]);
        break;
      case L2S_ACT_SWISH:
#pragma unroll
        for (int e = 0; e < 8; ++e) v[e] = l2s_swish(v[e]);
        break;
      case L2S_ACT_PRELU:
#pragma unroll
        for (int e = 0; e < 8; ++e) v[e] = v[e] >= 0.f ? v[e] : v[e] * sv[e];
        break;
      case L2S_ACT_LRELU:
#pragma unroll
        for (int e = 0; e < 8; ++e) v[e] = v[e] >= 0.f ? v[e] : v[e] * p.act_slope;
        break;
      case L2S_ACT_TANH:
#pragma unroll
        for (int e = 0; e < 8; ++e) v[e] = tanhf(v[e]);
        break;
      default: break;
    }
    }
    if (flags & L2S_F_RES_POST) {
#pragma unroll
      for (int e = 0; e < 8; ++e) v[e] += rv[e];
    }
    if (flags & L2S_F_ACCUM) {
#pragma unroll
      for (int e = 0; e < 8; ++e) v[e] += cv[e];
    }
    if (!keep) {
#pragma unroll
      for (int e = 0; e < 8; ++e) v[e] = 0.f;
    }
    if (flags & L2S_F_OUT_F32) {
      float* q = (float*)p.C + o * p.ldc + col;
      *reinterpret_cast<float4*>(q) = make_float4(v[0], v[1], v[2], v[3]);
      if (ok_hi) *reinterpret_cast<float4*>(q + 4) = make_float4(v[4], v[5], v[6], v[7]);
    } else {
      st8_16(p.C, o, p.ldc, v);
    }
    if (flags & L2S_F_DUAL) {
      float w[8];
#pragma unroll
      for (int e = 0; e < 8; ++e) w[e] = v[e] * p.slope2;
      if (p.slope2 > 0.f && p.slope2 <= 1.f) {
#pragma unroll
        for (int e = 0; e < 8; ++e) w[e] = fmaxf(v[e], w[e]);
      } else {
#pragma unroll
        for (int e = 0; e < 8; ++e) w[e] = v[e] >= 0.f ? v[e] : w[e];
      }
      st8_16(p.C2, o, p.ldc2, w);
    }
    }
  }
  if (MI > CH) asm volatile("" ::: "memory");
  };
  do_chunk(std::integral_constant<int, 0>{});
  if constexpr (MI > CH) do_chunk(std::integral_constant<int, CH>{});
  if constexpr (MI > 2 * CH) do_chunk(std::integral_constant<int, 2 * CH>{});
  if constexpr (MI > 3 * CH) do_chunk(std::integral_constant<int, 3 * CH>{});
  static_assert(MI <= 4 * CH, "chunk list");
}

template <typename ET, int MI, int NI, int ACTK, bool MASKED, int G2MAX = 2, typename RowMap>
// ... 250 lines not shown
          for (int e = 0; e < 8; ++e) v[e] += rv[e];
        }
        if constexpr (ACTK == 2) {
#ifdef L2S_GELU_ERF
#pragma unroll
          for (int e = 0; e < 8; ++e) v[e] = l2s_gelu(v[e]);
#else
#pragma unroll
          for (int e = 0; e < 8; e += 2) { const f32x2_t g = l2s_gelu2(f32x2_t{v[e], v[e + 1]}); v[e] = g.x; v[e + 1] = g.y; }
#endif
        } else if constexpr (ACTK == 1) {
          if (LEAN && act == L2S_ACT_LRELU && p.act_slope > 0.f && p.act_slope <= 1.f) {
            const float s_l = p.act_slope;
#pragma unroll
            for (int e = 0; e < 8; ++e) v[e] = fmaxf(v[e], v[e] * s_l);
          } else if (LEAN && act == L2S_ACT_RELU) {
#pragma unroll
            for (int e = 0; e < 8; ++e) v[e] = fmaxf(v[e], 0.f);
          } else if (LEAN || act != L2S_ACT_NONE) {
#pragma unroll
            for (int e = 0; e < 8; ++e) v[e] = fmaxf(v[e], 0.f) + fminf(v[e], 0.f) * sj[2 * b + (e >> 2)][e & 3];
          }
        }
        if (CAN_RES && (flags & L2S_F_RES_POST)) {
#pragma unroll
          for (int e = 0; e < 8; ++e) v[e] += rv[e];
        }
        if (!keep[i]) {
#pragma unroll
          for (int e = 0; e < 8; ++e) v[e] = 0.f;
        }
        const uint4 pk = make_uint4(ET::pack2(v[0], v[1]), ET::pack2(v[2], v[3]), ET::pack2(v[4], v[5]), ET::pack2(v[6], v[7]));
        uint4 pk2 = make_uint4(0, 0, 0, 0);
        if (dual) {
          float w[8];
#pragma unroll
          for (int e = 0; e < 8; ++e) w[e] = v[e] * p.slope2;
          if (p.slope2 > 0.f && p.slope2 <= 1.f) {
#pragma unroll
            for (int e = 0; e < 8; ++e) w[e] = fmaxf(v[e], w[e]);
          } else {
#pragma unroll
            for (int e = 0; e < 8; ++e) w[e] = v[e] >= 0.f ? v[e] : w[e];
          }
          pk2 = make_uint4(ET::pack2(w[0], w[1]), ET::pack2(w[2], w[3]), ET::pack2(w[4], w[5]), ET::pack2(w[6], w[7]));
        }
        if constexpr (!FULL) {
          if (orow[i] >= 0 && okb[b]) {
            *reinterpret_cast<uint4*>((uint16_t*)p.C + (int64_t)orow[i] * p.ldc + col0 + 32 * b) = pk;
            if (dual) *reinterpret_cast<uint4*>((uint16_t*)p.C2 + (int64_t)orow[i] * p.ldc2 + col0 + 32 * b) = pk2;
          }
        } else {
          held[b & 1] = pk;
          held2[b & 1] = pk2;
          if (b & 1) {
            const bool lower = lm < 8;
            const uint4 got = dpp_row_ror8_u4(held[1]);
            const uint4 xa = lower ? held[0] : got, xb = lower ? got : held[0];
            const int hA = lm >> 3, hB = 1 - hA;
            const int cA = col0 + 32 * (b - 1) + 32 * hA, cB = col0 + 32 * (b - 1) + 32 * hB;
            const int oa = (int)rowmap(row_base + (c0 + i) * 16 + (lm & 7)), ob = (int)rowmap(row_base + (c0 + i) * 16 + 8 + (lm & 7));
            const bool okA = oa >= 0 && (hA ? okb[b] : okb[b - 1]), okB = ob >= 0 && (hB ? okb[b] : okb[b - 1]);
            if (okA) *reinterpret_cast<uint4*>((uint16_t*)p.C + (int64_t)oa * p.ldc + cA) = xa;
            if (okB) *reinterpret_cast<uint4*>((uint16_t*)p.C + (int64_t)ob * p.ldc + cB) = xb;
            if (dual) {
              const uint4 got2 = dpp_row_ror8_u4(held2[1]);
              const uint4 ya = lower ? held2[0] : got2, yb = lower ? got2 : held2[0];
              if (okA) *reinterpret_cast<uint4*>((uint16_t*)p.C2 + (int64_t)oa * p.ldc2 + cA) = ya;
              if (okB) *reinterpret_cast<uint4*>((uint16_t*)p.C2 + (int64_t)ob * p.ldc2 + cB) = yb;
            }
          }
        }
      }
      if (c0 == 0 && i == 0) after_loads();
    }
  };
  do_chunk(std::integral_constant<int, 0>{});
  if constexpr (MI > CHK) do_chunk(std::integral_constant<int, CHK>{});
  if constexpr (MI > 2 * CHK) do_chunk(std::integral_constant<int, 2 * CHK>{});
  if constexpr (MI > 3 * CHK) do_chunk(std::integral_constant<int, 3 * CHK>{});
  static_assert(MI <= 4 * CHK, "chunk list");
}

__device__ __forceinline__ f32x4_t dpp_row_ror8(f32x4_t v) {
  float r0, r1, r2, r3;
  asm volatile("s_nop 1\n\tv_mov_b32_dpp %0, %4 row_ror:8 row_mask:0xf bank_mask:0xf\n\t"
               "v_mov_b32_dpp %1, %5 row_ror:8 row_mask:0xf bank_mask:0xf\n\t"
               "v_mov_b32_dpp %2, %6 row_ror:8 row_mask:0xf bank_mask:0xf\n\t"
               "v_mov_b32_dpp %3, %7 row_ror:8 row_mask:0xf bank_mask:0xf"
               : "=&v"(r0), "=&v"(r1), "=&v"(r2), "=&v"(r3)
               : "v"(v[0]), "v"(v[1]), "v"(v[2]), "v"(v[3]));
  return f32x4_t{r0, r1, r2, r3};
}

template <typename ET, int MI, int NI, typename RowMap>
__device__ __forceinline__ void epilogue_stream32(const l2s_gemm_desc& p, f32x4_t (&acc)[MI][NI], const int lane,
                                                  const int row_base, const int ncol_base, RowMap rowmap) {
  static_assert(MI % 2 == 0 && MI >= 4 && NI % 2 == 0, "row groups are streamed in pairs, two pairs in flight; blocks in pairs");
  constexpr int NB = NI / 2;
  const int lm = lane & 15, lg = lane >> 4;
  const bool lower = lm < 8;
  const float alpha = p.alpha;
  const char* __restrict__ rbase = (const char*)p.R;
  char* __restrict__ cbase = (char*)p.C;
  f32x4_t bj[NI];
#pragma unroll
  for (int j = 0; j < NI; ++j) {
    bj[j] = f32x4_t{0.f, 0.f, 0.f, 0.f};
    if (p.bias) { const float4 q = *reinterpret_cast<const float4*>(p.bias + ncol_base + j * 16 + lg * 4); bj[j] = f32x4_t{q.x, q.y, q.z, q.w}; }
  }
  const uint32_t colA = (uint32_t)(ncol_base + 16 * (lm >> 3) + lg * 4) * 4u;
  const uint32_t colB = (uint32_t)(ncol_base + 16 * (1 - (lm >> 3)) + lg * 4) * 4u;
  const uint32_t pitch = (uint32_t)p.ldc * 4u;
  const uint32_t gstep = 16u * (uint32_t)p.out_row_mul * pitch;
  const uint32_t offA0 = (uint32_t)rowmap(row_base + (lm & 7)) * pitch + colA;
  const uint32_t offB0 = (uint32_t)rowmap(row_base + 8 + (lm & 7)) * pitch + colB;
  auto ld = [&](uint32_t off) {
    const float4 q = *reinterpret_cast<const float4*>(rbase + (size_t)off);
    return f32x4_t{q.x, q.y, q.z, q.w};
  };
  auto st = [&](uint32_t off, f32x4_t v) { *reinterpret_cast<float4*>(cbase + (size_t)off) = make_float4(v[0], v[1], v[2], v[3]); };
  auto load_pair = [&](f32x4_t (&rv)[2][NB][2], auto pr_tag) {
    constexpr int pr = decltype(pr_tag)::value;
#pragma unroll
    for (int g = 0; g < 2; ++g)
#pragma unroll
      for (int b = 0; b < NB; ++b) {
        rv[g][b][0] = ld(offA0 + (uint32_t)(2 * pr + g) * gstep + (uint32_t)(b * 128));
        rv[g][b][1] = ld(offB0 + (uint32_t)(2 * pr + g) * gstep + (uint32_t)(b * 128));
      }
  };
  auto finish_pair = [&](f32x4_t (&rv)[2][NB][2], auto pr_tag) {
    constexpr int pr = decltype(pr_tag)::value;
#pragma unroll
    for (int g = 0; g < 2; ++g)
#pragma unroll
      for (int b = 0; b < NB; ++b) {
        const int i = 2 * pr + g;
        const f32x4_t u0 = (acc[i][2 * b] + bj[2 * b]) * alpha;
        const f32x4_t u1 = (acc[i][2 * b + 1] + bj[2 * b + 1]) * alpha;
        const f32x4_t got = dpp_row_ror8(u1);
        f32x4_t xa, xb;
#pragma unroll
        for (int e = 0; e < 4; ++e) { xa[e] = lower ? u0[e] : got[e]; xb[e] = lower ? got[e] : u0[e]; }
        st(offA0 + (uint32_t)i * gstep + (uint32_t)(b * 128), xa + rv[g][b][0]);
        st(offB0 + (uint32_t)i * gstep + (uint32_t)(b * 128), xb + rv[g][b][1]);
      }
  };
  f32x4_t ra[2][NB][2], rb[2][NB][2];
  load_pair(ra, std::integral_constant<int, 0>{});
  load_pair(rb, std::integral_constant<int, 1>{});
  finish_pair(ra, std::integral_constant<int, 0>{});
  if constexpr (MI > 4) load_pair(ra, std::integral_constant<int, 2>{});
  finish_pair(rb, std::integral_constant<int, 1>{});
  if constexpr (MI > 6) load_pair(rb, std::integral_constant<int, 3>{});
  if constexpr (MI > 4) finish_pair(ra, std::integral_constant<int, 2>{});
  if constexpr (MI > 6) finish_pair(rb, std::integral_constant<int, 3>{});
  static_assert(MI <= 8, "row group pairs");
}

template <typename ET, int MI, int NI, typename RowMap>
__device__ __forceinline__ void epilogue_stream32x(const l2s_gemm_desc& p, f32x4_t (&acc)[MI][NI], const int lane,
                                                   const int row_base, const int ncol_base, RowMap rowmap) {
  static_assert(MI % 2 == 0, "row groups are streamed in pairs");
  const int lm = lane & 15, lg = lane >> 4;
  const int flags = p.flags;
// ... 80 lines not shown
template <typename ET, int MI, int NI, typename RowMap>
__device__ __forceinline__ void epilogue_direct32(const l2s_gemm_desc& p, f32x4_t (&acc)[MI][NI], const int lane,
                                                  const int row_base, const int ncol_base, const int grp,
                                                  RowMap rowmap) {
#ifndef L2S_NO_STREAM32
  if constexpr (MI % 2 == 0 && MI >= 4) {
    if (grp == 0 && stream32_ok(p, row_base, ncol_base, MI * 16, NI * 16)) {
      epilogue_stream32<ET, MI, NI>(p, acc, lane, row_base, ncol_base, rowmap);
      return;
    }
  }
#endif
  const int lm = lane & 15, lg = lane >> 4;
  const int flags = p.flags;
  const bool has_res = (flags & (L2S_F_RES_PRE | L2S_F_RES_POST)) != 0;
  const float alpha = p.alpha;
  f32x4_t bj[NI], sj[NI];
  bool okj[NI];
#pragma unroll
  for (int j = 0; j < NI; ++j) {
    const int n = ncol_base + j * 16 + lg * 4;
    okj[j] = n < p.N;
    bj[j] = f32x4_t{0.f, 0.f, 0.f, 0.f};
    sj[j] = f32x4_t{0.f, 0.f, 0.f, 0.f};
    if (okj[j]) {
      if (p.bias) { const float4 q = *reinterpret_cast<const float4*>(p.bias + grp * p.N + n); bj[j] = f32x4_t{q.x, q.y, q.z, q.w}; }
      if (p.act == L2S_ACT_PRELU) { const float4 q = *reinterpret_cast<const float4*>(p.slope + grp * p.N + n); sj[j] = f32x4_t{q.x, q.y, q.z, q.w}; }
    }
    if (p.act != L2S_ACT_PRELU) {
      const float s_uni = p.act == L2S_ACT_RELU ? 0.f : (p.act == L2S_ACT_LRELU ? p.act_slope : 1.f);
      sj[j] = f32x4_t{s_uni, s_uni, s_uni, s_uni};
    }
  }
  auto do_group = [&](auto i_tag) {
    constexpr int i = decltype(i_tag)::value;
    const int o32 = (int)rowmap(row_base + i * 16 + lm);
    if (o32 < 0) return;
    const int64_t o = o32;
    f32x4_t rv[NI];
#pragma unroll
    for (int j = 0; j < NI; ++j) {
      rv[j] = f32x4_t{0.f, 0.f, 0.f, 0.f};
      if (has_res && okj[j]) {
        const int col = grp * p.c_gstride + ncol_base + j * 16 + lg * 4;
        if (flags & L2S_F_RES_F32) {
          const float4 q = *reinterpret_cast<const float4*>((const float*)p.R + o * p.ldr + col);
          rv[j] = f32x4_t{q.x, q.y, q.z, q.w};
        } else {
          const uint2 q = *reinterpret_cast<const uint2*>((const uint16_t*)p.R + o * p.ldr + col);
          rv[j] = f32x4_t{ET::to_f32((uint16_t)(q.x & 0xffff)), ET::to_f32((uint16_t)(q.x >> 16)),
                          ET::to_f32((uint16_t)(q.y & 0xffff)), ET::to_f32((uint16_t)(q.y >> 16))};
        }
      }
    }
#pragma unroll
    for (int j = 0; j < NI; ++j) {
      if (!okj[j]) continue;
      f32x4_t v = (acc[i][j] + bj[j]) * alpha;
      if (flags & L2S_F_RES_PRE) v = v + rv[j];
#pragma unroll
      for (int e = 0; e < 4; ++e) v[e] = fmaxf(v[e], 0.f) + fminf(v[e], 0.f) * sj[j][e];
      if (flags & L2S_F_RES_POST) v = v + rv[j];
      const int col = grp * p.c_gstride + ncol_base + j * 16 + lg * 4;
      *reinterpret_cast<float4*>((float*)p.C + o * p.ldc + col) = make_float4(v[0], v[1], v[2], v[3]);
    }
  };
  do_group(std::integral_constant<int, 0>{});
  if constexpr (MI > 1) do_group(std::integral_constant<int, 1>{});
  if constexpr (MI > 2) do_group(std::integral_constant<int, 2>{});
  if constexpr (MI > 3) do_group(std::integral_constant<int, 3>{});
  if constexpr (MI > 4) do_group(std::integral_constant<int, 4>{});
  if constexpr (MI > 5) do_group(std::integral_constant<int, 5>{});
  if constexpr (MI > 6) do_group(std::integral_constant<int, 6>{});
  if constexpr (MI > 7) do_group(std::integral_constant<int, 7>{});
  static_assert(MI <= 8, "row group list");
}

template <typename ET, int MI, int NI, int EPI, typename RowMap>
__device__ __forceinline__ void epilogue(const l2s_gemm_desc& p, f32x4_t (&acc)[MI][NI], const uint32_t scr,
                                         const int lane, const int row_base, const int ncol_base, const int grp,
                                         RowMap rowmap) {
  if constexpr (EPI < L2S_EPI_G16A)
    epilogue_fast16<ET, MI, NI, (EPI - L2S_EPI_F16) / 2, ((EPI - L2S_EPI_F16) & 1) != 0>(p, acc, scr, lane, row_base, ncol_base, grp, rowmap);
  else if constexpr (EPI == L2S_EPI_G16A) epilogue_impl<ET, MI, NI, F_G16A, true>(p, acc, scr, lane, row_base, ncol_base, grp, rowmap);
  else if constexpr (EPI == L2S_EPI_G16B) epilogue_impl<ET, MI, NI, F_G16B, true>(p, acc, scr, lane, row_base, ncol_base, grp, rowmap);
  else if constexpr (EPI == L2S_EPI_S32) {
#ifndef L2S_NO_STREAM32
    if constexpr (MI % 2 == 0 && MI >= 4) {
      if (grp == 0 && stream32_ok(p, row_base, ncol_base, MI * 16, NI * 16)) {
        epilogue_stream32<ET, MI, NI>(p, acc, lane, row_base, ncol_base, rowmap);
        return;
      }
    }
#endif
    epilogue_impl<ET, MI, NI, F_S32, true>(p, acc, scr, lane, row_base, ncol_base, grp, rowmap);
  }
  else epilogue_impl<ET, MI, NI, 0x7f, false>(p, acc, scr, lane, row_base, ncol_base, grp, rowmap);
}

}
```

lip2speech_unit_amd/csrc/tapgemm_f32.hip:

```cpp
#include "l2s_common.h"
#include <math.h>

namespace {

typedef __attribute__((ext_vector_type(16))) float f32x16_t;

constexpr int BM = 128, BN = 128, BK = 16;
constexpr int LDT = BM + 4;

template <int MODE>
__global__ __launch_bounds__(256, 2) void tapgemm_f32_kernel(const l2s_gemm_desc p, const int tiles_n) {
  __shared__ float sA[2][BK][LDT];
  __shared__ float sW[2][BK][LDT];
  const int tid = threadIdx.x, lane = tid & 63, wave = tid >> 6;
  const int grp = blockIdx.z;
  const int tile_m = blockIdx.x / tiles_n, tile_n = blockIdx.x - tile_m * tiles_n;
  const int m0 = tile_m * BM, n0 = tile_n * BN;
  const int Cin = p.Cin, Ktot = p.Cin * p.ntaps;
  const float* __restrict__ A = (const float*)p.A + (int64_t)grp * p.a_gstride;
  const float* __restrict__ W = (const float*)p.W + (int64_t)grp * p.w_gstride;

  const int ld_row = tid >> 2, ld_k = (tid & 3) * 4;
  const float* a_base[2];
  int a_t[2], a_x[2];
// ... 64 lines not shown
  f32x16_t acc[2][2];
#pragma unroll
  for (int i = 0; i < 2; ++i)
#pragma unroll
    for (int j = 0; j < 2; ++j)
#pragma unroll
      for (int e = 0; e < 16; ++e) acc[i][j][e] = 0.f;
  const int nk = (Ktot + BK - 1) / BK;
  fetch(0);
  stage(0);
  __syncthreads();
  for (int kt = 0; kt < nk; ++kt) {
    const int buf = kt & 1;
    if (kt + 1 < nk) fetch(kt + 1);
    if (wave_on) {
#pragma unroll
      for (int s = 0; s < BK / 2; ++s) {
        const int k = 2 * s + lh;
        const float a0 = sA[buf][k][wm + lr], a1 = sA[buf][k][wm + 32 + lr];
        const float w0 = sW[buf][k][wn + lr], w1 = sW[buf][k][wn + 32 + lr];
        acc[0][0] = __builtin_amdgcn_mfma_f32_32x32x2f32(a0, w0, acc[0][0], 0, 0, 0);
        acc[0][1] = __builtin_amdgcn_mfma_f32_32x32x2f32(a0, w1, acc[0][1], 0, 0, 0);
        acc[1][0] = __builtin_amdgcn_mfma_f32_32x32x2f32(a1, w0, acc[1][0], 0, 0, 0);
        acc[1][1] = __builtin_amdgcn_mfma_f32_32x32x2f32(a1, w1, acc[1][1], 0, 0, 0);
      }
    }
    if (kt + 1 < nk) stage(buf ^ 1);
    __syncthreads();
  }
  if (!wave_on) return;

  const int flags = p.flags, act = p.act;
  const float alpha = p.alpha;
  float* __restrict__ C = (float*)p.C;
  float* __restrict__ C2 = (float*)p.C2;
  const float* __restrict__ R = (const float*)p.R;
#pragma unroll
  for (int j = 0; j < 2; ++j) {
    const int n = n0 + wn + 32 * j + lr;
    if (n >= p.N) continue;
    const float bv = p.bias ? p.bias[grp * p.N + n] : 0.f;
    const float sv = act == L2S_ACT_PRELU ? p.slope[grp * p.N + n] : (act == L2S_ACT_LRELU ? p.act_slope : 0.f);
    const int col = grp * p.c_gstride + n;
#pragma unroll
    for (int i = 0; i < 2; ++i) {
#pragma unroll
      for (int e = 0; e < 16; ++e) {
        const int m = m0 + wm + 32 * i + 8 * (e >> 2) + 4 * lh + (e & 3);
        if (m >= p.M) continue;
        const int64_t o = (int64_t)m * p.out_row_mul + p.out_row_add;
        float v = acc[i][j][e] + bv;
        if (alpha != 1.f) v *= alpha;
        float rv = 0.f;
        if (flags & (L2S_F_RES_PRE | L2S_F_RES_POST)) rv = R[o * p.ldr + col];
        if (flags & L2S_F_RES_PRE) v += rv;
        switch (act) {
          case L2S_ACT_RELU: v = fmaxf(v, 0.f); break;
          case L2S_ACT_GELU: v = 0.5f * v * (1.0f + erff(v * 0.70710678118654752f)); break;
          case L2S_ACT_SWISH: v = v / (1.0f + expf(-v)); break;
          case L2S_ACT_PRELU:
          case L2S_ACT_LRELU: v = v >= 0.f ? v : v * sv; break;
          case L2S_ACT_TANH: v = tanhf(v); break;
          default: break;
        }
        if (flags & L2S_F_RES_POST) v += rv;
        if (flags & L2S_F_ACCUM) v += C[o * p.ldc + col];
        if (flags & L2S_F_MASK) {
          const int clip = (int)(o / p.mask_T);
          const int t = (int)(o - (int64_t)clip * p.mask_T);
          if (!(t < p.lens[clip] * p.mask_mul)) v = 0.f;
        }
        C[o * p.ldc + col] = v;
        if (flags & L2S_F_DUAL) C2[o * p.ldc2 + col] = v >= 0.f ? v : v * p.slope2;
      }
    }
  }
}

}

int l2s_tapgemm_f32_launch(const l2s_gemm_desc& d, hipStream_t st) {
  if (d.ktab) return L2S_EUNSUPPORTED;
  if (d.mode < 0 || d.mode > 2) return L2S_EINVAL;
  if ((d.Cin & 3) || (d.lda & 3) || (d.a_gstride & 3) || (d.w_gstride & 3)) return L2S_EALIGN;
  const int64_t tiles_m = ((int64_t)d.M + BM - 1) / BM, tiles_n = (d.N + BN - 1) / BN;
  if (tiles_m * tiles_n >= ((int64_t)1 << 31) || d.groups > 65535) return L2S_EUNSUPPORTED;
  dim3 grid((unsigned)(tiles_m * tiles_n), 1, (unsigned)d.groups), blk(256);
  if (d.mode == L2S_MODE_LINEAR) hipLaunchKernelGGL(tapgemm_f32_kernel<L2S_MODE_LINEAR>, grid, blk, 0, st, d, (int)tiles_n);
  else if (d.mode == L2S_MODE_CONV1D) hipLaunchKernelGGL(tapgemm_f32_kernel<L2S_MODE_CONV1D>, grid, blk, 0, st, d, (int)tiles_n);
  else hipLaunchKernelGGL(tapgemm_f32_kernel<L2S_MODE_CONV2D>, grid, blk, 0, st, d, (int)tiles_n);
  L2S_CHECK_LAUNCH();
  return L2S_OK;
}
```

lip2speech_unit_amd/csrc/tapgemm_tiles.h:

```cpp
#pragma once
#include <cstdlib>

namespace l2s {
struct TileCfg { int bm, bn; float eff; };
inline int pick_tile(int M, int N, int G) {
  auto cdiv = [](int a, int b) { return (a + b - 1) / b; };
  static const int forced = [] { const char* e = getenv("L2S_FORCE_TILE"); return e ? atoi(e) : 0; }();
  if (forced) return forced;
  if (N <= 16) return 128016;
  if (N <= 32) return 128032;
  static const TileCfg cands[] = {{256, 128, 1.0f}, {256, 64, 0.8f}, {128, 128, 0.8f}, {128, 64, 0.62f}, {64, 64, 0.4f}};
  int best = 0;
  float best_cost = 1e30f;
  for (const TileCfg& c : cands) {
    if (c.bn == 128 && N < 128) continue;
    const long nt = (long)cdiv(M, c.bm) * cdiv(N, c.bn) * G;
    const float cost = (float)cdiv((int)nt, 256) * (float)(c.bm * c.bn) / c.eff;
    if (cost < best_cost) { best_cost = cost; best = c.bm * 1000 + c.bn; }
  }
  return best;
}

enum { L2S_EPI_F16 = 0,
       L2S_EPI_G16A = 6,
       L2S_EPI_G16B = 7,
       L2S_EPI_S32 = 8,
       L2S_EPI_ALL = 9,
       L2S_EPI_COUNT = 10,
       L2S_EPI_X32 = 10 };
inline bool is_x32(int flags, int act) {
  const int need = 0x2  | 0x20 , may = 0x4  | 0x8  | 0x10 ;
  return act == 0 && (flags & need) == need && (flags & ~(need | may)) == 0;
}
inline int pick_epilogue(int flags, int act) {
  const bool lin = act == 0  || act == 1  || act == 4  || act == 5 ;
  if ((flags & ~0x10) == 0) {
    const int m = (flags & 0x10) ? 1 : 0;
    if (act == 0) return L2S_EPI_F16 + 0 + m;
    if (lin) return L2S_EPI_F16 + 2 + m;
    if (act == 2 ) return L2S_EPI_F16 + 4 + m;
    return L2S_EPI_ALL;
  }
  if ((flags & ~(0x1 | 0x2)) == 0 && lin) return L2S_EPI_G16A;
  if ((flags & ~(0x1 | 0x2 | 0x8 | 0x10)) == 0 && lin) return L2S_EPI_G16B;
  if ((flags & ~(0x1 | 0x2 | 0x20 | 0x40)) == 0 && (flags & 0x20) && lin) return L2S_EPI_S32;
  return L2S_EPI_ALL;
}

}
```

lip2speech_unit_amd/ops.py:

```python
import ctypes
import os
from typing import Optional

import torch

from . import _lib
from ._lib import (ACT_GELU, ACT_LRELU, ACT_NONE, ACT_PRELU, ACT_RELU, ACT_SWISH, ACT_TANH, BF16, F16, F32, F_ACCUM,
                   F_DUAL, F_MASK, F_OUT_F32, F_RES_F32, F_RES_POST, F_RES_PRE, MODE_CONV1D, MODE_CONV2D,
                   MODE_LINEAR, GemmDesc, L2SError, check)

_TORCH16 = {F16: torch.float16, BF16: torch.bfloat16, F32: torch.float32}
_DTYPE_NAME = {F16: "f16", BF16: "bf16", F32: "f32"}


class KernelProfiler:

    def __init__(self, detail=False):
        self.records = []
        self.detail = detail

    def summary(self):
        torch.cuda.synchronize()
        agg = {}
        for key, fl, by, e0, e1, shape in self.records:
            a = agg.setdefault(key, {"calls": 0, "ms": 0.0, "flops": 0.0, "bytes": 0.0, "shapes": {}})
            ms = e0.elapsed_time(e1)
            for t in (a, a["shapes"].setdefault(shape, {"calls": 0, "ms": 0.0, "flops": 0.0, "bytes": 0.0})):
                t["calls"] += 1
                t["ms"] += ms
                t["flops"] += fl
                t["bytes"] += by
        return agg


_profiler = None


def set_profiler(p):
    global _profiler
    _profiler = p


def _run(key, call, flops=0.0, nbytes=0.0, shape=None):
    if _profiler is None:
        return check(call(), key)
    e0, e1 = torch.cuda.Event(enable_timing=True), torch.cuda.Event(enable_timing=True)
    e0.record()
    rc = call()
    e1.record()
    check(rc, key)
    _profiler.records.append((key, flops, nbytes, e0, e1, shape))


def torch_dtype(dtype: int) -> torch.dtype:
    return _TORCH16[dtype]


def dtype_code(t: torch.dtype) -> int:
    if t == torch.float16:
        return F16
    if t == torch.bfloat16:
        return BF16
    if t == torch.float32:
        return F32
    raise L2SError(f"unsupported operand dtype {t}")


def _stream() -> int:
    return torch.cuda.current_stream().cuda_stream


def _ptr(t: Optional[torch.Tensor]) -> Optional[int]:
    if t is None:
        return None
    if not t.is_cuda:
        raise L2SError("HIP ops need device tensors (there is no CPU path)")
    return t.data_ptr()


def _req(t: torch.Tensor, dtype=None, name="tensor"):
    if not t.is_cuda:
        raise L2SError(f"{name}: expected a device tensor (there is no CPU path)")
    if dtype is not None and t.dtype != dtype:
        raise L2SError(f"{name}: expected {dtype}, got {t.dtype}")
    if t.dim() >= 2 and t.stride(-1) != 1:
        raise L2SError(f"{name}: innermost dim must be contiguous")
    return t


def _extent(t: torch.Tensor) -> int:
    if t.numel() == 0:
        return 0
    return 1 + sum((n - 1) * st for n, st in zip(t.shape, t.stride()))


def tapgemm(A, W, C, *, M, N, Cin, ntaps=1, lda=None, ldc=None, bias=None, slope=None, R=None, ldr=None, C2=None,
            ldc2=None, lens=None, mode=MODE_LINEAR, T_out=0, T_in=0, stride=1, dil=1, off=0, Ho=0, Wo=0, Hi=0, Wi=0,
            KW=1, pad=0, out_row_mul=1, out_row_add=0, mask_T=0, mask_mul=1, act=ACT_NONE, flags=0, dtype=F16,
            alpha=1.0, act_slope=0.0, slope2=0.0, groups=1, a_gstride=0, c_gstride=0, w_gstride=0, ktab=None, kflops=None):
    lib = _lib.load()
    d = GemmDesc()
    d.A, d.W, d.C = _ptr(A), _ptr(W), _ptr(C)
    d.C2, d.bias, d.slope, d.R, d.lens = _ptr(C2), _ptr(bias), _ptr(slope), _ptr(R), _ptr(lens)
    if bias is not None and bias.dtype != torch.float32:
        raise L2SError("bias must be fp32")
    if lens is not None and lens.dtype != torch.int32:
        raise L2SError("lens must be int32")
    d.M, d.N, d.Cin, d.ntaps = M, N, Cin, ntaps
    d.lda = lda if lda is not None else Cin
    d.ldc = ldc if ldc is not None else N * groups
    d.ldc2 = ldc2 if ldc2 is not None else d.ldc
    d.ldr = ldr if ldr is not None else d.ldc
    d.mode = mode
    d.T_out, d.T_in, d.stride, d.dil, d.off = T_out, T_in, stride, dil, off
    d.Ho, d.Wo, d.Hi, d.Wi, d.KW, d.pad = Ho, Wo, Hi, Wi, KW, pad
    d.out_row_mul, d.out_row_add = out_row_mul, out_row_add
    d.mask_T, d.mask_mul = mask_T, mask_mul
    if C.dtype == torch.float32:
        flags |= F_OUT_F32
    if R is not None and R.dtype == torch.float32:
        flags |= F_RES_F32
    d.act, d.flags, d.dtype = act, flags, dtype
    d.alpha, d.act_slope, d.slope2 = alpha, act_slope, slope2
    d.groups, d.a_gstride, d.c_gstride, d.w_gstride = groups, a_gstride, c_gstride, w_gstride
    if ktab is not None:
        if ktab.dtype != torch.int32 or ktab.dim() != 2 or ktab.shape != (groups, 20) or not ktab.is_contiguous():
            raise L2SError("ktab: int32 [groups, 20], contiguous")
        d.ktab = _ptr(ktab)
    if _profiler is None:
        check(lib.l2s_tapgemm(ctypes.byref(d), _stream()), "l2s_tapgemm")
        return
    var = lib.l2s_tapgemm_variant(ctypes.byref(d))
    key = f"tapgemm<{_DTYPE_NAME[dtype]},{var // 1000 % 1000}x{var % 1000},mode{mode}>"
    if _profiler is not None:
        fam = lib.l2s_tapgemm_epilogue_family(ctypes.byref(d))
        if var in (999064, 999128):
            fam = {0: 2, 1: 3, 2: 2, 3: 3, 6: 6, 7: 7}.get(fam, 9)
        key = key[:-1] + f",e{fam}>"
    if _profiler is not None and _profiler.detail:
        key += f" M{M} N{N} Cin{Cin} taps{ntaps} g{groups} fl{flags:#x} act{act} alpha{alpha:g}"
    ktot = Cin * ntaps
    osz = 4 if dtype == F32 else 2
    esz = 4 if (flags & F_OUT_F32) else osz
    mn = float(M) * N * groups
    nbytes = float(osz) * M * ktot * groups / max(ntaps, 1) + float(osz) * N * ktot * groups + esz * mn
    if R is not None:
        nbytes += (4 if (flags & F_RES_F32) else osz) * mn
    if flags & F_DUAL:
        nbytes += osz * mn
    if flags & F_ACCUM:
        nbytes += esz * mn
    _run(key, lambda: lib.l2s_tapgemm(ctypes.byref(d), _stream()), kflops if kflops is not None else 2.0 * M * N * ktot * groups, nbytes,
         shape=f"M{M} N{N * groups} K{ktot}" + (" ktab" if ktab is not None else ""))


def stem_conv3d(x, w, bias, slope, y, B, T, dtype):
    lib = _lib.load()
    _run("l2s_stem_conv3d", lambda: lib.l2s_stem_conv3d(_ptr(x), int(x.dtype == torch.float32), _ptr(w), _ptr(bias), _ptr(slope), _ptr(y), B, T,
                              x.shape[-2], x.shape[-1], dtype, _stream()))


def stem_pool_fused(x, w, bias, slope, y, B, T, dtype):
    lib = _lib.load()
    _run("l2s_stem_pool_fused", lambda: lib.l2s_stem_pool_fused(
        _ptr(x), int(x.dtype == torch.float32), _ptr(w), _ptr(bias), _ptr(slope), _ptr(y), B, T, x.shape[-2], x.shape[-1],
        dtype, _stream()), flops=2.0 * B * T * 44 * 44 * 64 * 245,
        nbytes=B * T * (88 * 88 * (4 if x.dtype == torch.float32 else 2) + 22 * 22 * 64 * 2))


def stem_pool_fused_u8(frames, w, bias, slope, y, B, T, dtype, crop=88, mean=0.421, std=0.165):
    lib = _lib.load()
    if frames.dtype != torch.uint8 or frames.dim() != 4:
        raise ValueError("frames: uint8 [B,T,Hin,Win]")
    Hin, Win = frames.shape[-2], frames.shape[-1]
    _run("l2s_stem_pool_fused", lambda: lib.l2s_stem_pool_fused_u8(
        _ptr(frames), Hin, Win, crop, mean, std, _ptr(w), _ptr(bias), _ptr(slope), _ptr(y), B, T, dtype, _stream()),
        flops=2.0 * B * T * 44 * 44 * 64 * 245, nbytes=B * T * (crop * crop + 22 * 22 * 64 * 2))


def maxpool2d_3x3s2(x, y, N, H, W, C, dtype):
    _run("l2s_maxpool2d_3x3s2", lambda: _lib.load().l2s_maxpool2d_3x3s2(_ptr(x), _ptr(y), N, H, W, C, dtype, _stream()))


def avgpool_hw(x, y, N, HW, C, dtype):
    _run("l2s_avgpool_hw", lambda: _lib.load().l2s_avgpool_hw(_ptr(x), _ptr(y), N, HW, C, dtype, _stream()))


def layernorm(x, gamma, beta, eps, y, *, M, C, ldx=None, ldy=None, y2=None, ldy2=0, zero_prefix=0, lens=None,
              len_mul=1, mask_T=0, dtype=F16):
    ldx = ldx if ldx is not None else C
    ldy = ldy if ldy is not None else C + zero_prefix
    _run("l2s_layernorm", lambda: _lib.load().l2s_layernorm(_ptr(x), int(x.dtype == torch.float32), ldx, _ptr(gamma), _ptr(beta), eps, _ptr(y),
                                    int(y.dtype == torch.float32), ldy, _ptr(y2), ldy2, M, C, zero_prefix,
                                    _ptr(lens), len_mul, mask_T, dtype, _stream()))


def attention(qkv, out, *, B, T, H, ldq=None, ldo=None, pos=None, ldp=0, bias_u=None, bias_v=None, lens=None,
              len_mul=1, dtype=F16):
    ldq = ldq if ldq is not None else 3 * H * 64
    ldo = ldo if ldo is not None else H * 64
    _run("l2s_attention", lambda: _lib.load().l2s_attention(_ptr(qkv), ldq, _ptr(out), ldo, _ptr(pos), ldp, _ptr(bias_u), _ptr(bias_v),
                                    _ptr(lens), len_mul, B, T, H, dtype, _stream()))


def glu_dwconv_swish(x, w, bias, y, *, B, T, C, k, lens=None, len_mul=1, dtype=F16):
    _run("l2s_glu_dwconv_swish", lambda: _lib.load().l2s_glu_dwconv_swish(_ptr(x), _ptr(w), _ptr(bias), _ptr(y), _ptr(lens), len_mul, B, T, C, k,
                                           dtype, _stream()))


def greedy_decode(logits, tokens, lprobs, score, *, B, T2, V, ldl=None, lens=None, len_mul=1, temperature=1.0,
                  lenpen=1.0):
    ldl = ldl if ldl is not None else V
    _run("l2s_greedy_decode", lambda: _lib.load().l2s_greedy_decode(_ptr(logits), ldl, _ptr(lens), len_mul, B, T2, V, temperature, lenpen,
                                        _ptr(tokens), _ptr(lprobs), _ptr(score), _stream()))


def beam_decode(logits, *, B, T2, V, beam, ldl=None, lens=None, len_mul=1, temperature=1.0, lenpen=1.0):
    lib = _lib.load()
    dev = logits.device
    ldl = ldl if ldl is not None else V
    nbytes = lib.l2s_beam_decode_workspace(B, T2, beam)
    if nbytes == 0:
        raise L2SError("l2s_beam_decode_workspace: bad shape")
    work = torch.empty(nbytes, device=dev, dtype=torch.uint8)
    tokens = torch.empty(B, beam, T2 + 1, device=dev, dtype=torch.int32)
    pos = torch.empty(B, beam, T2 + 1, device=dev, dtype=torch.float32)
    score = torch.empty(B, beam, device=dev, dtype=torch.float32)
    nhyp = torch.empty(B, device=dev, dtype=torch.int32)
    _run("l2s_beam_decode", lambda: lib.l2s_beam_decode(_ptr(_req(logits, torch.float32, "logits")), ldl, _ptr(lens), len_mul, B, T2, V,
                                                          temperature, lenpen, beam, _ptr(work), nbytes, _ptr(tokens), _ptr(pos),
                                                          _ptr(score), _ptr(nhyp), _stream()))
    return tokens, pos, score, nhyp


def ctc_frames(logits, labels, topk_cls, topk_lp, *, B, L, V, K, ldl=None, lens=None, len_mul=1):
    ldl = ldl if ldl is not None else V
    _run("l2s_ctc_frames", lambda: _lib.load().l2s_ctc_frames(
        _ptr(_req(logits, torch.float32, "logits")), ldl, _ptr(lens), len_mul, B, L, V, K, _ptr(_req(labels, torch.int32, "labels")),
        _ptr(topk_cls), _ptr(topk_lp), _stream()))


def ctc_beam_search(topk_cls, topk_lp, workspace, labels, lengths, scores, *, B, L, K, beam, nbest, lens=None, len_mul=1):
    _run("l2s_ctc_beam_search", lambda: _lib.load().l2s_ctc_beam_search(
        _ptr(_req(topk_cls, torch.int32, "topk_cls")), _ptr(_req(topk_lp, torch.float32, "topk_lp")), _ptr(lens), len_mul, B, L, K,
        beam, nbest, _ptr(workspace), workspace.numel() * workspace.element_size(), _ptr(_req(labels, torch.int32, "labels")),
        _ptr(_req(lengths, torch.int32, "lengths")), _ptr(_req(scores, torch.float32, "scores")), _stream()))


def ctc_repeat_labels(x, y, *, B, L, ldx=None, ldy=None, lens=None, len_mul=1):
    _run("l2s_ctc_repeat_labels", lambda: _lib.load().l2s_ctc_repeat_labels(
        _ptr(_req(x, torch.int32, "x")), ldx or x.stride(0), _ptr(lens), len_mul, B, L, _ptr(_req(y, torch.int32, "y")),
        ldy or y.stride(0), _stream()))


def ctc_beam_workspace_bytes(B, L, beam):
    n = _lib.load().l2s_ctc_beam_workspace(B, L, beam)
    if n == 0:
        raise L2SError(f"l2s_ctc_beam_workspace: unsupported size (B={B}, L={L}, beam={beam})")
    return n


def ctc_decode(logits, *, B, L, V, ldl=None, lens=None, len_mul=1, beam=0, K=40, nbest=3):
    dev = logits.device
    labels = torch.empty(B, L, device=dev, dtype=torch.int32)
    if beam <= 0:
        ctc_frames(logits, labels, None, None, B=B, L=L, V=V, K=0, ldl=ldl, lens=lens, len_mul=len_mul)
        return {"text": labels}
    K = min(K, V)
    nbest = min(nbest, beam)
    tc = torch.empty(B, L, K, device=dev, dtype=torch.int32)
    tl = torch.empty(B, L, K, device=dev, dtype=torch.float32)
    ctc_frames(logits, labels, tc, tl, B=B, L=L, V=V, K=K, ldl=ldl, lens=lens, len_mul=len_mul)
    work = torch.empty(ctc_beam_workspace_bytes(B, L, beam) // 8, device=dev, dtype=torch.int64)
    beams = torch.empty(B, nbest, L, device=dev, dtype=torch.int32)
    blen = torch.empty(B, nbest, device=dev, dtype=torch.int32)
    bsc = torch.empty(B, nbest, device=dev, dtype=torch.float32)
    ctc_beam_search(tc, tl, work, beams, blen, bsc, B=B, L=L, K=K, beam=beam, nbest=nbest, lens=lens, len_mul=len_mul)
    return {"text": labels, "text_beams": beams, "text_lens": blen, "text_scores": bsc}


def repeat2_cast(x, y, B, T, C, dtype):
    _run("l2s_repeat2_cast", lambda: _lib.load().l2s_repeat2_cast(_ptr(x), _ptr(y), B, T, C, dtype, _stream()))


def splitk_reduce(P, x, *, M, N, S, ldp=None, ldx=None):
    _run("l2s_splitk_reduce", lambda: _lib.load().l2s_splitk_reduce(_ptr(P), ldp or S * N, S, _ptr(x), ldx or N, M, N, _stream()))


SPLITK_MAX_M = 512
_SPLITK_ON = os.environ.get("L2S_SPLITK", "1") != "0"
# ... 400 lines not shown
        _ptr(x), ldx, N, _ptr(rows), M, _ptr(centers), _ptr(cnorm), D, K, _ptr(ids), _ptr(dmin), _ptr(inertia), _ptr(workspace),
        _ws_bytes(workspace) if workspace is not None else 0, _stream()),
        flops=2.0 * M * K * D, nbytes=4.0 * M * D + 4.0 * K * D + 8.0 * M)


def kmeans_update(x, ids, centers, counts, centers_out, counts_out, cnorm_out, workspace, *, M, D, K, rows=None, ldx=None):
    ldx, N = _km_batch("kmeans_update", x, rows, M, D, ldx)
    _req(ids, torch.int32, "ids"), _req(workspace, None, "workspace")
    for t, nm, n in ((centers, "centers", K * D), (counts, "counts", K), (centers_out, "centers_out", K * D), (counts_out, "counts_out", K),
                     (cnorm_out, "cnorm_out", K)):
        _req(t, torch.float32, nm)
        if t.numel() < n or not t.is_contiguous():
            raise L2SError(f"kmeans_update: {nm} dense with {n} elements")
    if ids.numel() < M or not ids.is_contiguous():
        raise L2SError("kmeans_update: ids shorter than M")
    _run("l2s_kmeans_update", lambda: _lib.load().l2s_kmeans_update(
        _ptr(x), ldx, N, _ptr(rows), M, _ptr(ids), _ptr(centers), _ptr(counts), D, K, _ptr(centers_out), _ptr(counts_out),
        _ptr(cnorm_out), _ptr(workspace), _ws_bytes(workspace), _stream()), flops=1.0 * M * D, nbytes=4.0 * M * D + 8.0 * K * D + 8.0 * M)


def kmeans_pp_pot(x, cand, workspace, *, m, D, t, rows=None, closest=None, select=None, pot=None, closest_out=None, chosen=None,
                  ldx=None):
    ldx, N = _km_batch("kmeans_pp_pot", x, rows, m, D, ldx)
    _req(cand, torch.int32, "cand"), _req(workspace, None, "workspace")
    n_pot = 1 if closest_out is not None else t
    for a, dt, nm, n in ((closest, torch.float32, "closest", m), (select, torch.float64, "select", t), (pot, torch.float64, "pot", n_pot),
                         (closest_out, torch.float32, "closest_out", m), (chosen, torch.int32, "chosen", 1)):
        if a is not None:
            _req(a, dt, nm)
            if a.numel() < n or not a.is_contiguous():
                raise L2SError(f"kmeans_pp_pot: {nm} shorter than {n}")
    if cand.numel() < t or not cand.is_contiguous():
        raise L2SError("kmeans_pp_pot: cand shorter than t")
    _run("l2s_kmeans_pp_pot", lambda: _lib.load().l2s_kmeans_pp_pot(
        _ptr(x), ldx, N, _ptr(rows), m, D, _ptr(cand), t, _ptr(closest), _ptr(select), _ptr(pot), _ptr(closest_out), _ptr(chosen),
        _ptr(workspace), _ws_bytes(workspace), _stream()), flops=3.0 * m * D * n_pot, nbytes=4.0 * m * D + 8.0 * m)


def kmeans_pp_pick(closest, u, idx, *, m, t, scale=None, total=None):
    _req(closest, torch.float32, "closest"), _req(u, torch.float64, "u"), _req(idx, torch.int32, "idx")
    for a, nm in ((scale, "scale"), (total, "total")):
        if a is not None:
            _req(a, torch.float64, nm)
            if a.numel() < 1:
                raise L2SError(f"kmeans_pp_pick: {nm} is empty")
    if closest.numel() < m or not closest.is_contiguous() or u.numel() < t or idx.numel() < t:
        raise L2SError("kmeans_pp_pick: closest shorter than m / u, idx shorter than t")
    _run("l2s_kmeans_pp_pick", lambda: _lib.load().l2s_kmeans_pp_pick(
        _ptr(closest), m, _ptr(u) if t else None, t, _ptr(scale), _ptr(idx), _ptr(total), _stream()), nbytes=4.0 * m * (1 + t))


_TG = ("(Tensor A, Tensor W, Tensor(a!) C, *, int M, int N, int Cin, int ntaps=1, int? lda=None, int? ldc=None, Tensor? bias=None, "
       "Tensor? slope=None, Tensor? R=None, int? ldr=None, Tensor(b!)? C2=None, int? ldc2=None, Tensor? lens=None, int mode=0, "
       "int T_out=0, int T_in=0, int stride=1, int dil=1, int off=0, int Ho=0, int Wo=0, int Hi=0, int Wi=0, int KW=1, int pad=0, "
       "int out_row_mul=1, int out_row_add=0, int mask_T=0, int mask_mul=1, int act=0, int flags=0, int dtype=0, float alpha=1.0, "
       "float act_slope=0.0, float slope2=0.0, int groups=1, int a_gstride=0, int c_gstride=0, int w_gstride=0, Tensor? ktab=None, "
       "float? kflops=None) -> ()")
_ATT = ("(Tensor qkv, Tensor(a!) out, *, int B, int T, int H, int? ldq=None, int? ldo=None, Tensor? pos=None, int ldp=0, "
        "Tensor? bias_u=None, Tensor? bias_v=None, Tensor? lens=None, int len_mul=1, int dtype=0) -> ()")
_STEM = "(Tensor x, Tensor w, Tensor bias, Tensor? slope, Tensor(a!) y, int B, int T, int dtype) -> ()"
_RP = ("(Tensor x_l, Tensor w1, Tensor b1, Tensor w2, Tensor b2, *, int B, int T, int C, int k, int dil, float slope, "
       "Tensor(a!)? y=None, Tensor(b!)? xs=None, bool accumulate=False, Tensor? lens=None, int len_mul=1, int dtype=0, "
       "bool xs_final=True) -> ()")
_CPT = ("(Tensor x, Tensor w, float bias, Tensor(a!) wav, Tensor(b!)? pcm, *, int B, int T, int C, int k, Tensor? lens=None, "
        "int len_mul=1) -> ()")
_GLU = ("(Tensor x, Tensor w, Tensor bias, Tensor(a!) y, *, int B, int T, int C, int k, Tensor? lens=None, int len_mul=1, "
        "int dtype=0) -> ()")
_LN = ("(Tensor x, Tensor gamma, Tensor beta, float eps, Tensor(a!) y, *, int M, int C, int? ldx=None, int? ldy=None, "
       "Tensor(b!)? y2=None, int ldy2=0, int zero_prefix=0, Tensor? lens=None, int len_mul=1, int mask_T=0, int dtype=0) -> ()")
_GD = ("(Tensor logits, Tensor(a!) tokens, Tensor(b!) lprobs, Tensor(c!) score, *, int B, int T2, int V, int? ldl=None, "
       "Tensor? lens=None, int len_mul=1, float temperature=1.0, float lenpen=1.0) -> ()")
_BL = "(Tensor x, Tensor[] ws, Tensor[] biases, Tensor[] slopes, Tensor(a!) y, *, int n_images, int H, int W, int C=64, int dtype=0) -> ()"
_SCHEMAS = {
    "tapgemm": _TG,
    "stem_conv3d": _STEM,
    "stem_pool_fused": _STEM,
    "stem_pool_fused_u8": "(Tensor frames, Tensor w, Tensor bias, Tensor? slope, Tensor(a!) y, int B, int T, int dtype, int crop=88, "
                          "float mean=0.421, float std=0.165) -> ()",
    "maxpool2d_3x3s2": "(Tensor x, Tensor(a!) y, int N, int H, int W, int C, int dtype) -> ()",
    "avgpool_hw": "(Tensor x, Tensor(a!) y, int N, int HW, int C, int dtype) -> ()",
    "layernorm": _LN,
    "attention": _ATT,
    "glu_dwconv_swish": _GLU,
    "greedy_decode": _GD,
    "beam_decode": "(Tensor logits, *, int B, int T2, int V, int beam, int? ldl=None, Tensor? lens=None, int len_mul=1, "
                   "float temperature=1.0, float lenpen=1.0) -> (Tensor, Tensor, Tensor, Tensor)",
    "repeat2_cast": "(Tensor x, Tensor(a!) y, int B, int T, int C, int dtype) -> ()",
    "ctc_frames": "(Tensor logits, Tensor(a!) labels, Tensor(b!)? topk_cls, Tensor(c!)? topk_lp, *, int B, int L, int V, int K, "
                  "int? ldl=None, Tensor? lens=None, int len_mul=1) -> ()",
    "ctc_repeat_labels": "(Tensor x, Tensor(a!) y, *, int B, int L, int? ldx=None, int? ldy=None, Tensor? lens=None, "
                         "int len_mul=1) -> ()",
    "ctc_beam_search": "(Tensor topk_cls, Tensor topk_lp, Tensor(a!) workspace, Tensor(b!) labels, Tensor(c!) lengths, "
                       "Tensor(d!) scores, *, int B, int L, int K, int beam, int nbest, Tensor? lens=None, int len_mul=1) -> ()",
    "splitk_reduce": "(Tensor P, Tensor(a!) x, *, int M, int N, int S, int? ldp=None, int? ldx=None) -> ()",
    "splitk_reduce_layernorm": "(Tensor P, Tensor(a!) x, Tensor gamma, Tensor beta, float eps, Tensor(b!) y, *, int M, int C, int S, "
                               "int? ldp=None, int? ldx=None, int? ldy=None, Tensor? lens=None, int len_mul=1, int mask_T=0, int dtype=0) -> ()",
    "cast_f32_to_16": "(Tensor x, Tensor(a!) y, int M, int C, int dtype, int? ldx=None, int? ldy=None) -> ()",
    "cast_16_to_f32": "(Tensor x, Tensor(a!) y, int M, int C, int dtype, int? ldx=None, int? ldy=None) -> ()",
    "broadcast_rows": "(Tensor v, Tensor(a!) y, *, int B, int T, int C, int ldy, int col0=0, int? ldv=None, Tensor? lens=None, "
                      "int len_mul=1, int dtype=0) -> ()",
    "transpose_ct_to_tc": "(Tensor x, Tensor(a!) y, *, int B, int C, int T, int ldy, int col0=0, Tensor? lens=None, int len_mul=1, "
                          "int dtype=0) -> ()",
    "embedding": "(Tensor code, Tensor table, Tensor(a!) y, *, int B, int L, int C, int? ldy=None, Tensor? lens=None, int dtype=0) -> ()",
    "embedding_tokens": "(Tensor tok, Tensor table, Tensor(a!) y, *, int B, int L, int C, int token_offset=4, int? ldt=None, "
                        "int? ldy=None, Tensor? lens=None, int len_mul=1, int dtype=0) -> ()",
    "rows_f32_to_16_masked": "(Tensor x, Tensor(a!) y, *, int B, int T, int C, int? ldx=None, int? ldy=None, int col0=0, "
                             "Tensor? lens=None, int len_mul=1, int dtype=0) -> ()",
    "lens_from_mask": "(Tensor? padding_mask, int B, int T, Device device) -> Tensor",
    "basicblock_fused": "(Tensor x, Tensor w1, Tensor b1, Tensor s1, Tensor w2, Tensor b2, Tensor s2, Tensor(a!) y, *, int n_images, "
                        "int H, int W, int C=64, int dtype=0) -> ()",
    "basiclayer_fused": _BL,
    "basicstage128_tail_fused": "(Tensor x0, Tensor t0, Tensor wa, Tensor ba, Tensor sa, Tensor w1, Tensor b1, Tensor s1, Tensor w2, "
                                "Tensor b2, Tensor s2, Tensor(a!) y, *, int n_images, int H, int W, int dtype=0) -> ()",
    "split_hi_lo": "(Tensor x, Tensor(a!) hi, Tensor(b!) lo, *, int B, int T, int C, int act=0, float slope=0.0, int? ldx=None, "
                   "int? ld16=None, Tensor? lens=None, int len_mul=1, int dtype=0) -> ()",
    "conv_post_tanh": _CPT,
    "resblock_fused": "(Tensor xl, Tensor w, Tensor bias, Tensor(a!) xs, Tensor(b!)? xl_out, *, int B, int T, int C, int k, int[] dil, "
                      "bool accumulate, float slope, Tensor? lens=None, int len_mul=1, int dtype=0) -> ()",
    "resstage_fused": "(Tensor xl, Tensor[] ws, Tensor[] biases, Tensor(a!) xs, Tensor(b!)? xl_out, *, int B, int T, int C, int[] ks, "
                      "int[] dils, float slope, Tensor? lens=None, int len_mul=1, int dtype=0, bool xs_final=True) -> ()",
    "respair": _RP,
    "respair_final": "(Tensor[] xs_l, Tensor[] w1s, Tensor[] b1s, Tensor[] w2s, Tensor[] b2s, Tensor(a!) y, *, int B, int T, int C, int[] ks, "
                     "int[] dils, float slope, Tensor? lens=None, int len_mul=1, int dtype=0) -> ()",
    "preprocess_frames": "(Tensor frames, Tensor(a!) y, *, int B, int T, int Hin, int Win, int crop=88, float mean=0.421, "
                         "float std=0.165, int dtype=0) -> ()",
    "mel_spectrogram": "(Tensor wav, Tensor(a!) mel, Tensor basis, Tensor fb, Tensor fb_range, *, int B, int S, int T_rows, "
                       "Tensor? n_samples=None, int? ldw=None, int? ldm=None, int n_fft=640, int hop=160, int n_mels=80, "
                       "float floor=1e-05) -> ()",
    "stft_mel": "(Tensor wav, Tensor(a!) mel, Tensor basis, Tensor fb, Tensor fb_range, *, int B, int S, int T_rows, int n_fft, int hop, "
                "int pad, float mag_eps=0.0, Tensor? n_samples=None, int? ldw=None, int? ldm=None, int n_mels=80, "
                "float floor=1e-05) -> ()",
    "unit_ce": "(Tensor logits, Tensor target, Tensor(a!) nll, Tensor(b!) smooth, Tensor(c!) n_correct, Tensor(d!) n_tok, *, int B, "
               "int T2, int V, int? ldl=None, int? ldt=None, Tensor? lens=None, int len_mul=2, int pad_idx=1, "
               "int ignore_prefix=0) -> ()",
    "mel_l1_sc": "(Tensor pred, Tensor targ, Tensor(a!) l1, Tensor(b!) sq, Tensor(c!) tsq, Tensor(d!) n_rows, *, int B, int Tm_pred, "
                 "int Tm_targ, int crop_len, Tensor? lens=None, int len_mul=4, int n_mels=80) -> ()",
    "ctc_loss": "(Tensor logits, Tensor targets, Tensor tgt_lens, Tensor tgt_offs, Tensor(a!) workspace, Tensor(b!) nll, *, int B, "
                "int L, int V, int S_max, int blank=0, int? ldl=None, Tensor? lens=None, int len_mul=2) -> ()",
    "wave_stem": "(Tensor wav, Tensor w, Tensor gamma, Tensor beta, Tensor(a!) workspace, Tensor(b!) out, *, int B, int S, int T_rows, "
                 "int C=512, Tensor? n_samples=None, int? ldw=None, int? ldo=None, float eps=1e-05, int dtype=0) -> ()",
    "kmeans_assign": "(Tensor x, Tensor centers, Tensor cnorm, Tensor(a!) ids, *, int B, int T, int D, int K, int? ldx=None, "
                     "Tensor? lens=None, int len_mul=1, Tensor(b!)? best2=None) -> ()",
    "kmeans_nearest": "(Tensor x, Tensor centers, Tensor cnorm, *, int M, int D, int K, Tensor? rows=None, Tensor(a!)? ids=None, "
                      "Tensor(b!)? dmin=None, Tensor(c!)? inertia=None, Tensor(d!)? workspace=None, int? ldx=None) -> ()",
    "kmeans_update": "(Tensor x, Tensor ids, Tensor centers, Tensor counts, Tensor(a!) centers_out, Tensor(b!) counts_out, "
                     "Tensor(c!) cnorm_out, Tensor(d!) workspace, *, int M, int D, int K, Tensor? rows=None, int? ldx=None) -> ()",
    "kmeans_pp_pot": "(Tensor x, Tensor cand, Tensor(a!) workspace, *, int m, int D, int t, Tensor? rows=None, Tensor? closest=None, "
                     "Tensor? select=None, Tensor(b!)? pot=None, Tensor(c!)? closest_out=None, Tensor(d!)? chosen=None, "
                     "int? ldx=None) -> ()",
    "kmeans_pp_pick": "(Tensor closest, Tensor u, Tensor(a!) idx, *, int m, int t, Tensor? scale=None, Tensor(b!)? total=None) -> ()",
}
ENTRY_OF = {n: "l2s_" + n for n in _SCHEMAS}
ENTRY_OF.update({"maxpool2d_3x3s2": "l2s_maxpool2d_3x3s2", "avgpool_hw": "l2s_avgpool_hw"})
HOST_QUERIES = ("l2s_abi_version", "l2s_build_info", "l2s_tapgemm_variant", "l2s_tapgemm_epilogue_family", "l2s_beam_decode_workspace",
                "l2s_ctc_beam_workspace", "l2s_ctc_loss_workspace", "l2s_wave_stem_workspace", "l2s_kmeans_nearest_workspace",
                "l2s_kmeans_update_workspace", "l2s_kmeans_pp_workspace")
ALIASES = {"frontend3d_stem": "stem_pool_fused", "resnet_trunk": "basiclayer_fused", "linear_epilogue": "tapgemm",
           "posconv_gelu": "tapgemm", "convtranspose1d": "tapgemm", "mel_head": "tapgemm", "mhsa_padmask": "attention",
           "relpos_mhsa": "attention", "conformer_conv_module": "glu_dwconv_swish", "greedy_unit_decode": "greedy_decode",
           "resblock1": "respair", "tanh_to_int16": "conv_post_tanh"}

_TORCH_LIB = torch.library.Library("lip2speech", "DEF")


def _fake_none(*a, **k):
    return None
# ... 61 lines not shown
```

Baseline: 13500.

## Fuse GLU into pointwise conv GEMM epilogue and add plain dwconv-swish kernel

Interleaves the value and gate rows of the first pointwise conv's weights and bias so each lane holds adjacent value/gate columns. A new GLU epilogue in the tapgemm and phasegemm paths then applies the sigmoid gate and writes only half-width output. A new LDS-pipelined depthwise conv + swish kernel consumes that gated tensor instead of redoing GLU. This is meant to halve the intermediate write and read traffic between the GEMM and the depthwise conv, at the cost of new epilogue code paths, remapped weight-load indexing in the paired phase GEMM, and an extra copy of the pw1 weights.

```diff
diff --git a/include/lip2speech_hip.h b/include/lip2speech_hip.h
--- a/include/lip2speech_hip.h
+++ b/include/lip2speech_hip.h
@@ -21,7 +21,8 @@
   L2S_ACT_SWISH = 3,
   L2S_ACT_PRELU = 4,
   L2S_ACT_LRELU = 5,
-  L2S_ACT_TANH = 6
+  L2S_ACT_TANH = 6,
+  L2S_ACT_GLU = 7
 };
 
 enum {
@@ -99,6 +100,9 @@
 int l2s_glu_dwconv_swish(const void* x, const float* w, const float* bias, void* y, const int32_t* lens,
                          int len_mul, int B, int T, int C, int k, int dtype, void* stream);
 
+int l2s_dwconv_swish(const void* u, const float* w, const float* bias, void* y, const int32_t* lens, int len_mul, int B,
+                     int T, int C, int k, int dtype, int max_blocks, void* stream);
+
 int l2s_greedy_decode(const float* logits, int ldl, const int32_t* lens, int len_mul, int B, int T2, int V,
                       float temperature, float lenpen, int32_t* tokens, float* lprobs, float* score, void* stream);
 
diff --git a/lip2speech_unit_amd/_lib.py b/lip2speech_unit_amd/_lib.py
--- a/lip2speech_unit_amd/_lib.py
+++ b/lip2speech_unit_amd/_lib.py
@@ -6,6 +6,7 @@
 
 F16, BF16, F32 = 0, 1, 2
 ACT_NONE, ACT_RELU, ACT_GELU, ACT_SWISH, ACT_PRELU, ACT_LRELU, ACT_TANH = range(7)
+ACT_GLU = 7
 F_RES_PRE, F_RES_POST, F_ACCUM, F_DUAL, F_MASK, F_OUT_F32, F_RES_F32 = (1 << i for i in range(7))
 MODE_LINEAR, MODE_CONV1D, MODE_CONV2D = 0, 1, 2
 ABI_VERSION = 16
@@ -71,6 +72,7 @@
     "l2s_layernorm": ([_vp, _i, _i, _vp, _vp, _f, _vp, _i, _i, _vp, _i, _i, _i, _i, _vp, _i, _i, _i, _vp], _i),
     "l2s_attention": ([_vp, _i, _vp, _i, _vp, _i, _vp, _vp, _vp, _i, _i, _i, _i, _i, _vp], _i),
     "l2s_glu_dwconv_swish": ([_vp, _vp, _vp, _vp, _vp, _i, _i, _i, _i, _i, _i, _vp], _i),
+    "l2s_dwconv_swish": ([_vp, _vp, _vp, _vp, _vp, _i, _i, _i, _i, _i, _i, _i, _vp], _i),
     "l2s_greedy_decode": ([_vp, _i, _vp, _i, _i, _i, _i, _f, _f, _vp, _vp, _vp, _vp], _i),
     "l2s_beam_decode": ([_vp, _i, _vp, _i, _i, _i, _i, _f, _f, _i, _vp, ctypes.c_size_t, _vp, _vp, _vp, _vp, _vp], _i),
     "l2s_beam_decode_workspace": ([_i, _i, _i], ctypes.c_size_t),
diff --git a/lip2speech_unit_amd/conformer.py b/lip2speech_unit_amd/conformer.py
--- a/lip2speech_unit_amd/conformer.py
+++ b/lip2speech_unit_amd/conformer.py
@@ -6,7 +6,18 @@
 import torch.nn as nn
 
 from . import ops
-from .ops import ACT_GELU, ACT_RELU, F_MASK, F_RES_POST, MODE_CONV1D
+from .ops import ACT_GELU, ACT_GLU, ACT_RELU, F_MASK, F_RES_POST, MODE_CONV1D
+
+GLU_EPI = os.environ.get("L2S_GLU_EPI", "1") != "0"
+
+
+def glu_interleave(t):
+    C = t.shape[0] // 2
+    return torch.stack([t[:C], t[C:]], 1).reshape(t.shape)
+
+
+def glu_deinterleave(t):
+    return torch.cat([t[0::2], t[1::2]], 0)
 
 
 @dataclass
@@ -170,6 +181,8 @@
                 "v": (a.pos_bias_v.detach().float() * inv).to(dev).contiguous(),
                 "wo": w16(a.linear_out.weight), "bo": _f32(a.linear_out.bias, dev),
                 "pw1": w16(c.pointwise_cov1.weight[:, :, 0]), "pb1": _f32(c.pointwise_cov1.bias, dev),
+                "pw1g": w16(glu_interleave(c.pointwise_cov1.weight.detach()[:, :, 0])),
+                "pb1g": _f32(glu_interleave(c.pointwise_cov1.bias.detach()), dev),
                 "dw": dw.t().contiguous().to(dev), "db": db.to(dev).contiguous(),
                 "pw2": w16(c.pointwise_cov2.weight[:, :, 0]), "pb2": _f32(c.pointwise_cov2.bias, dev),
                 "n_ffm": _ln(L.norm_ff_macaron, dev), "n_mha": _ln(L.norm_mha, dev), "n_conv": _ln(L.norm_conv, dev),
@@ -212,7 +225,8 @@
         f = torch.empty(M, F, device=dev, dtype=t16)
         qkv = torch.empty(M, 3 * d, device=dev, dtype=t16)
         att = torch.empty(M, d, device=dev, dtype=t16)
-        glu_in = torch.empty(M, 2 * d, device=dev, dtype=t16)
+        glu_epi = GLU_EPI and dt != ops.F32 and not self.raven
+        glu_in = torch.empty(M, d if glu_epi else 2 * d, device=dev, dtype=t16)
         cv = torch.empty(M, d, device=dev, dtype=t16)
 
         def half_ffn(e, name, norm, after, y):
@@ -239,8 +253,12 @@
                           lens=lens, len_mul=len_mul, dtype=dt)
             ops.tapgemm(att, e["wo"], x, M=M, N=d, Cin=d, bias=e["bo"], R=x, ldr=d, flags=F_RES_POST, dtype=dt)
             ops.layernorm(x, e["n_conv"][0], e["n_conv"][1], 1e-12, h, M=M, C=d, dtype=dt)
-            ops.tapgemm(h, e["pw1"], glu_in, M=M, N=2 * d, Cin=d, bias=e["pb1"], dtype=dt)
-            ops.glu_dwconv_swish(glu_in, e["dw"], e["db"], cv, B=B, T=T, C=d, k=k, lens=lens, len_mul=len_mul, dtype=dt)
+            if glu_epi:
+                ops.tapgemm(h, e["pw1g"], glu_in, M=M, N=2 * d, Cin=d, bias=e["pb1g"], act=ACT_GLU, dtype=dt)
+                ops.dwconv_swish(glu_in, e["dw"], e["db"], cv, B=B, T=T, C=d, k=k, lens=lens, len_mul=len_mul, dtype=dt)
+            else:
+                ops.tapgemm(h, e["pw1"], glu_in, M=M, N=2 * d, Cin=d, bias=e["pb1"], dtype=dt)
+                ops.glu_dwconv_swish(glu_in, e["dw"], e["db"], cv, B=B, T=T, C=d, k=k, lens=lens, len_mul=len_mul, dtype=dt)
             ops.tapgemm(cv, e["pw2"], x, M=M, N=d, Cin=d, bias=e["pb2"], R=x, ldr=d, flags=F_RES_POST, dtype=dt)
             half_ffn(e, "ff", e["n_ff"], e["n_fin"], x)
         return x
diff --git a/lip2speech_unit_amd/csrc/conformer_conv.hip b/lip2speech_unit_amd/csrc/conformer_conv.hip
--- a/lip2speech_unit_amd/csrc/conformer_conv.hip
+++ b/lip2speech_unit_amd/csrc/conformer_conv.hip
@@ -1,4 +1,5 @@
 #include "l2s_common.h"
+#include "tapgemm_common.h"
 
 namespace {
 
@@ -75,3 +76,198 @@
   L2S_CHECK_LAUNCH();
   return L2S_OK;
 }
+
+namespace {
+
+using namespace l2s;
+
+template <int OPT>
+struct DwCfg {
+  static constexpr int TT = 8 * OPT;
+  static constexpr int ROWS = TT + KMAX - 1;
+  static constexpr int NDMA = (ROWS + 63) / 64;
+  static constexpr int BUF_B = NDMA * 8 * 1024;
+  static constexpr int OUT_B = TT * CT * 2;
+  static constexpr int SMEM = 2 * BUF_B + OUT_B;
+  static constexpr int NST = (TT * 8 + 511) / 512;
+};
+
+__device__ __forceinline__ uint32_t lds_read_u16(uint32_t addr, const int off) {
+  uint32_t v;
+  asm volatile("ds_read_u16 %0, %1 offset:%2" : "=v"(v) : "v"(addr), "n"(off));
+  return v;
+}
+__device__ __forceinline__ void lds_write_b16(uint32_t addr, uint32_t v, const int off) {
+  asm volatile("ds_write_b16 %0, %1 offset:%2" ::"v"(addr), "v"(v), "n"(off) : "memory");
+}
+
+template <typename ET, int OPT>
+__global__ __launch_bounds__(512) void dwconv_swish_kernel(const uint16_t* __restrict__ u, const float* __restrict__ w,
+                                                           const float* __restrict__ bias, uint16_t* __restrict__ y,
+                                                           const int32_t* __restrict__ lens, int len_mul, int B, int T, int C,
+                                                           int k, int tiles, int gsplit) {
+  using Cfg = DwCfg<OPT>;
+  constexpr int TT = Cfg::TT, NDMA = Cfg::NDMA, NST = Cfg::NST;
+  extern __shared__ __attribute__((aligned(16))) uint16_t dw_lds[];
+  const int tid = threadIdx.x, lane = tid & 63;
+  const int wave = __builtin_amdgcn_readfirstlane(tid >> 6);
+  const int c = lane, tq = wave;
+  const int half = (k - 1) / 2, rows_k = TT + k - 1;
+  const int per_g = B * tiles;
+  const uint16_t* zero = reinterpret_cast<const uint16_t*>(&g_zero16);
+  typedef const int32_t __attribute__((address_space(4)))* clens_t;
+  const clens_t clens = (clens_t)(uintptr_t)lens;
+  const uint32_t lds_base = (uint32_t)(uintptr_t)(lptr_t)dw_lds;
+  const uint32_t out_base = lds_base + 2 * Cfg::BUF_B;
+  const int nb = (int)gridDim.x / gsplit;
+  const int glane = (int)blockIdx.x % gsplit, slot = (int)blockIdx.x / gsplit;
+  const int my_n = slot < per_g ? (per_g - 1 - slot) / nb + 1 : 0;
+  if (my_n == 0) return;
+
+  auto limit = [&](int i) {
+    if (i >= my_n) return 0;
+    const int b = (slot + i * nb) / tiles;
+    const int lim = lens ? clens[b] * len_mul : T;
+    return lim < T ? lim : T;
+  };
+  for (int g = glane; g < C / CT; g += gsplit) {
+    float wr[KMAX];
+#pragma unroll
+    for (int j = 0; j < KMAX; ++j) wr[j] = j < k ? w[j * C + g * CT + c] : 0.f;
+    float bs = bias[g * CT + c];
+#pragma unroll
+    for (int j = 0; j < KMAX; ++j) asm volatile("" : "+v"(wr[j]));
+    asm volatile("" : "+v"(bs));
+    const uint16_t* ug = u + g * CT + (lane & 7) * 8;
+    auto stage = [&](int i, int lim_i) {
+      const int idx = i < my_n ? slot + i * nb : 0;
+      const int b = idx / tiles, t0 = (idx - b * tiles) * TT;
+      uint16_t* dst = dw_lds + (i & 1) * (Cfg::BUF_B / 2);
+      const uint16_t* src = ug + ((int64_t)b * T) * C;
+#pragma unroll
+      for (int j = 0; j < NDMA; ++j) {
+        const int q = j * 8 + wave;
+        const int r = q * 8 + (lane >> 3);
+        const int t = t0 - half + r;
+        const bool ok = r < rows_k && (unsigned)t < (unsigned)lim_i;
+        const uint16_t* gsrc = ok ? src + (int64_t)t * C : zero;
+        __builtin_amdgcn_global_load_lds((gptr_t)gsrc, (lptr_t)(dst + q * 512), 16, 0, 0);
+      }
+    };
+    uint32_t pend_row0 = 0;
+    int pend_n = 0;
+    auto flush = [&]() {
+      u32x4_t d[NST];
+#pragma unroll
+      for (int n = 0; n < NST; ++n) {
+        const int ch = tid + n * 512;
+        d[n] = lds_read_u4(out_base + (uint32_t)(ch < TT * 8 ? ch : TT * 8 - 1) * 16u);
+      }
+      lds_wait();
+#pragma unroll
+      for (int n = 0; n < NST; ++n) {
+        const int ch = tid + n * 512, r = ch >> 3;
+        if (r < pend_n)
+          *reinterpret_cast<uint4*>(y + ((int64_t)pend_row0 + r) * C + g * CT + (ch & 7) * 8) = make_uint4(d[n].x, d[n].y, d[n].z, d[n].w);
+      }
+    };
+
+    int lim = limit(0), lim_nx = limit(1);
+    stage(0, lim);
+    for (int i = 0; i < my_n; ++i) {
+      const int idx = slot + i * nb;
+      const int b = idx / tiles, t0 = (idx - b * tiles) * TT;
+      stage(i + 1, lim_nx);
+      const int lim_n2 = limit(i + 2);
+      __builtin_amdgcn_sched_barrier(0);
+      wait_vmcnt<NDMA>();
+      asm volatile("" ::: "memory");
+      __builtin_amdgcn_s_barrier();
+      asm volatile("" ::: "memory");
+      const uint32_t wbase = lds_base + (uint32_t)((i & 1) * Cfg::BUF_B) + (uint32_t)((tq * OPT) * CT + c) * 2u;
+      uint32_t raw[OPT + KMAX - 1];
+#pragma unroll
+      for (int j = 0; j < OPT + KMAX - 1; ++j) raw[j] = lds_read_u16(wbase, j * CT * 2);
+      lds_wait();
+      float win[OPT + KMAX - 1];
+#pragma unroll
+      for (int j = 0; j < OPT + KMAX - 1; ++j) win[j] = (tq * OPT + j < rows_k) ? ET::to_f32((uint16_t)raw[j]) : 0.f;
+      if (pend_n > 0) flush();
+      uint32_t res[OPT];
+#pragma unroll
+      for (int o = 0; o < OPT; ++o) {
+        const int t = t0 + tq * OPT + o;
+        float acc = bs;
+#pragma unroll
+        for (int j = 0; j < KMAX; ++j) acc += win[o + j] * wr[j];
+        acc = l2s_swish(acc);
+        res[o] = ET::from_f32(t < lim ? acc : 0.f);
+      }
+      asm volatile("" ::: "memory");
+      __builtin_amdgcn_s_barrier();
+      asm volatile("" ::: "memory");
+      const uint32_t obase = out_base + (uint32_t)((tq * OPT) * CT + c) * 2u;
+#pragma unroll
+      for (int o = 0; o < OPT; ++o) lds_write_b16(obase, res[o], o * CT * 2);
+      asm volatile("s_waitcnt lgkmcnt(0)" ::: "memory");
+      pend_row0 = (uint32_t)(b * T + t0);
+      pend_n = T - t0 < TT ? T - t0 : TT;
+      lim = lim_nx;
+      lim_nx = lim_n2;
+    }
+    asm volatile("" ::: "memory");
+    __builtin_amdgcn_s_barrier();
+    asm volatile("" ::: "memory");
+    flush();
+    wait_vmcnt<0>();
+    asm volatile("" ::: "memory");
+    __builtin_amdgcn_s_barrier();
+    asm volatile("" ::: "memory");
+  }
+}
+
+template <typename ET, int OPT>
+int launch_dwconv(const void* u, const float* w, const float* bias, void* y, const int32_t* lens, int len_mul, int B, int T, int C,
+                  int k, int max_blocks, hipStream_t st) {
+  using Cfg = DwCfg<OPT>;
+  auto kern = dwconv_swish_kernel<ET, OPT>;
+  static L2sSmemOptIn opt_in;
+  if (int e = l2s_smem_opt_in(kern, Cfg::SMEM, opt_in)) return e;
+  const int tiles = (T + Cfg::TT - 1) / Cfg::TT;
+  const int64_t per_g = (int64_t)B * tiles;
+  if (per_g >= ((int64_t)1 << 30) || (int64_t)B * T >= ((int64_t)1 << 31)) return L2S_EUNSUPPORTED;
+  static const int cus = [] {
+    int dev = 0, n = 0;
+    if (hipGetDevice(&dev) != hipSuccess || hipDeviceGetAttribute(&n, hipDeviceAttributeMultiprocessorCount, dev) != hipSuccess || n <= 0) n = 256;
+    return n;
+  }();
+  int budget = cus;
+  if (max_blocks > 0 && budget > max_blocks) budget = max_blocks;
+  const int G = C / CT;
+  const int gsplit = G < budget ? G : budget;
+  int64_t nb = budget / gsplit;
+  if (nb > per_g) nb = per_g;
+  hipLaunchKernelGGL(kern, dim3((unsigned)(gsplit * nb)), dim3(512), Cfg::SMEM, st, (const uint16_t*)u, w, bias, (uint16_t*)y, lens,
+                     len_mul, B, T, C, k, tiles, gsplit);
+  L2S_CHECK_LAUNCH();
+  return L2S_OK;
+}
+
+}
+
+extern "C" int l2s_dwconv_swish(const void* u, const float* w, const float* bias, void* y, const int32_t* lens, int len_mul,
+                                int B, int T, int C, int k, int dtype, int max_blocks, void* stream) {
+  if (!u || !w || !bias || !y) return L2S_EINVAL;
+  if (B <= 0 || T <= 0 || C <= 0) return L2S_ESHAPE;
+  if (k <= 0 || k > KMAX || !(k & 1)) return L2S_EUNSUPPORTED;
+  if (C % CT) return L2S_EALIGN;
+  if (((uintptr_t)u & 15) || ((uintptr_t)y & 15)) return L2S_EALIGN;
+  if (dtype != L2S_F16 && dtype != L2S_BF16) return dtype == L2S_F32 ? L2S_EUNSUPPORTED : L2S_EINVAL;
+  hipStream_t st = (hipStream_t)stream;
+  const bool small = T <= 200;
+  if (dtype == L2S_F16)
+    return small ? launch_dwconv<ElemF16, 25>(u, w, bias, y, lens, len_mul, B, T, C, k, max_blocks, st)
+                 : launch_dwconv<ElemF16, 32>(u, w, bias, y, lens, len_mul, B, T, C, k, max_blocks, st);
+  return small ? launch_dwconv<ElemBF16, 25>(u, w, bias, y, lens, len_mul, B, T, C, k, max_blocks, st)
+               : launch_dwconv<ElemBF16, 32>(u, w, bias, y, lens, len_mul, B, T, C, k, max_blocks, st);
+}
diff --git a/lip2speech_unit_amd/csrc/phasegemm.hip b/lip2speech_unit_amd/csrc/phasegemm.hip
--- a/lip2speech_unit_amd/csrc/phasegemm.hip
+++ b/lip2speech_unit_amd/csrc/phasegemm.hip
@@ -33,6 +33,7 @@
   static const int res_on = [] { const char* e = getenv("L2S_PHASEGEMM_RES"); return e ? atoi(e) : 1; }();
   if (!res_on && (fam == l2s::L2S_EPI_G16A || fam == l2s::L2S_EPI_G16B)) return false;
   if (fam == l2s::L2S_EPI_S32 && ((d.ldc & 3) || (d.ldr & 3))) return false;
+  if (fam == l2s::L2S_EPI_GLU && (d.mode != L2S_MODE_LINEAR || (d.ldc & 7))) return false;
   if ((d.Cin % 64) || d.N < 256 || d.M < 256 || (d.lda & 7)) return false;
   if (d.mode == L2S_MODE_LINEAR && ((d.M & 7) || (d.N & 7))) return false;
   if (mode == 2) return true;
diff --git a/lip2speech_unit_amd/csrc/phasegemm_kernel.h b/lip2speech_unit_amd/csrc/phasegemm_kernel.h
--- a/lip2speech_unit_amd/csrc/phasegemm_kernel.h
+++ b/lip2speech_unit_amd/csrc/phasegemm_kernel.h
@@ -27,9 +27,9 @@
   constexpr int MODE = KT ? (int)L2S_MODE_LINEAR : MODE_T;
   constexpr int MI = 8, NI = 4;
 #ifdef L2S_NO_PAIRED
-  constexpr bool PAIRED = false;
+  constexpr bool PAIRED = EPI == L2S_EPI_GLU;
 #else
-  constexpr bool PAIRED = EPI <= L2S_EPI_G16A;
+  constexpr bool PAIRED = EPI <= L2S_EPI_G16A || EPI == L2S_EPI_GLU;
 #endif
   extern __shared__ __attribute__((aligned(16))) uint16_t lds[];
   const int tid = threadIdx.x, lane = tid & 63;
@@ -113,6 +113,7 @@
           mg = mg < p.M ? mg : p.M - 8;
           sa_base[h][j] = (const char*)p.A + (int64_t)mg * p.lda * 2;
           int ng = n0 + (wave >> 1) * 64 + h * 32 + 16 * (wave & 1) + 8 * j;
+          if constexpr (EPI == L2S_EPI_GLU) ng = n0 + (wave >> 1) * 64 + 16 * (2 * (wave & 1) + j) + 8 * h;
           ng = ng < p.N ? ng : p.N - 8;
           sw_base[h][j] = (const char*)p.W + (int64_t)ng * K * 2;
         }
@@ -373,6 +374,8 @@
       epilogue_stream32x<ET, MI, NI>(p, acc, lane, m0 + wr * 128, n0 + wc * 64, rowmap);
     } else if constexpr (EPI == L2S_EPI_S32) {
       epilogue_direct32<ET, MI, NI>(p, acc, lane, m0 + wr * 128, n0 + wc * 64, grp, rowmap);
+    } else if constexpr (EPI == L2S_EPI_GLU) {
+      epilogue_glu_direct16<ET, MI, NI>(p, acc, lane, m0 + wr * 128, n0 + wc * 64, rowmap);
     } else if constexpr (PAIRED) {
       epilogue_direct16<ET, MI, NI, EPI, decltype(rowmap), NoHook, true>(p, acc, lane, m0 + wr * 128, n0 + wc * 64, grp, rowmap);
     } else if constexpr (EPI == L2S_EPI_G16A) {
@@ -449,6 +452,9 @@
       case L2S_EPI_G16A: return launch_phase<ET, MODE, L2S_EPI_G16A>(d, st);
       case L2S_EPI_G16B: return launch_phase<ET, MODE, L2S_EPI_G16B>(d, st);
       case L2S_EPI_S32: return launch_phase<ET, MODE, L2S_EPI_S32>(d, st);
+      case L2S_EPI_GLU:
+        if constexpr (MODE == L2S_MODE_LINEAR) return launch_phase<ET, MODE, L2S_EPI_GLU>(d, st);
+        else return L2S_EUNSUPPORTED;
       case L2S_EPI_ALL: return is_x32(d.flags, d.act) ? launch_phase<ET, MODE, L2S_EPI_X32>(d, st) : (int)L2S_EUNSUPPORTED;
       default: return L2S_EUNSUPPORTED;
     }
diff --git a/lip2speech_unit_amd/csrc/tapgemm.hip b/lip2speech_unit_amd/csrc/tapgemm.hip
--- a/lip2speech_unit_amd/csrc/tapgemm.hip
+++ b/lip2speech_unit_amd/csrc/tapgemm.hip
@@ -9,6 +9,7 @@
 #define L2S_DECL_MODE(m) L2S_DECL(m, 0) L2S_DECL(m, 1) L2S_DECL(m, 2) L2S_DECL(m, 3) L2S_DECL(m, 4) L2S_DECL(m, 5) \
                          L2S_DECL(m, 6) L2S_DECL(m, 7) L2S_DECL(m, 8) L2S_DECL(m, 9)
 L2S_DECL_MODE(0) L2S_DECL_MODE(1) L2S_DECL_MODE(2)
+L2S_DECL(0, 11)
 #undef L2S_DECL_MODE
 #undef L2S_DECL
 
@@ -22,6 +23,7 @@
 #undef L2S_ROW
 #undef L2S_E
   if (d.mode < 0 || d.mode > 2) return L2S_EINVAL;
+  if (d.act == L2S_ACT_GLU) return d.dtype == L2S_F16 ? l2s_tapgemm_f16_m0_e11(d, st) : l2s_tapgemm_bf16_m0_e11(d, st);
   return table[d.dtype == L2S_F16 ? 0 : 1][d.mode][l2s::pick_epilogue(d.flags, d.act)](d, st);
 }
 
@@ -43,6 +45,12 @@
   if (d.M <= 0 || d.N <= 0 || d.Cin <= 0 || d.ntaps <= 0) return L2S_ESHAPE;
   if (d.groups <= 0) d.groups = 1;
   if (d.out_row_mul <= 0) d.out_row_mul = 1;
+  if (d.act == L2S_ACT_GLU) {
+    if (d.dtype == L2S_F32 || d.mode != L2S_MODE_LINEAR || d.ntaps != 1 || d.groups != 1 || d.ktab || (d.flags & ~L2S_F_MASK) ||
+        d.out_row_mul != 1 || d.out_row_add != 0)
+      return L2S_EUNSUPPORTED;
+    if (d.N & 7) return L2S_EALIGN;
+  }
   if (d.dtype == L2S_F32) {
     if (((uintptr_t)d.A & 15) || ((uintptr_t)d.W & 15) || ((uintptr_t)d.C & 3)) return L2S_EALIGN;
     if ((d.flags & (L2S_F_RES_PRE | L2S_F_RES_POST)) && !d.R) return L2S_EINVAL;
diff --git a/lip2speech_unit_amd/csrc/tapgemm_common.h b/lip2speech_unit_amd/csrc/tapgemm_common.h
--- a/lip2speech_unit_amd/csrc/tapgemm_common.h
+++ b/lip2speech_unit_amd/csrc/tapgemm_common.h
@@ -71,7 +71,7 @@
 constexpr int F_G16B = L2S_F_RES_PRE | L2S_F_RES_POST | L2S_F_DUAL | L2S_F_MASK;
 constexpr int F_S32 = L2S_F_RES_PRE | L2S_F_RES_POST | L2S_F_OUT_F32 | L2S_F_RES_F32;
 
-template <typename ET, int MI, int NI, int FEAT, bool LIN, bool SWZ = false, typename RowMap>
+template <typename ET, int MI, int NI, int FEAT, bool LIN, bool SWZ = false, bool GLU = false, typename RowMap>
 __device__ __forceinline__ void epilogue_impl(const l2s_gemm_desc& p, f32x4_t (&acc)[MI][NI], const uint32_t scr,
                                               const int lane, const int row_base, const int ncol_base, const int grp,
                                               RowMap rowmap) {
@@ -241,6 +241,13 @@
     if (p.alpha != 1.f) {
 #pragma unroll
       for (int e = 0; e < 8; ++e) v[e] *= p.alpha;
+    }
+    if constexpr (GLU) {
+      float u[4];
+#pragma unroll
+      for (int q = 0; q < 4; ++q) u[q] = keep ? v[2 * q] * __builtin_amdgcn_rcpf(1.0f + __expf(-v[2 * q + 1])) : 0.f;
+      *reinterpret_cast<uint2*>((uint16_t*)p.C + o * p.ldc + (col >> 1)) = make_uint2(ET::pack2(u[0], u[1]), ET::pack2(u[2], u[3]));
+      continue;
     }
     if (flags & L2S_F_RES_PRE) {
 #pragma unroll
@@ -657,6 +664,63 @@
   static_assert(MI <= 4 * CHK, "chunk list");
 }
 
+template <typename ET, int MI, int NI, typename RowMap>
+__device__ __forceinline__ void epilogue_glu_direct16(const l2s_gemm_desc& p, f32x4_t (&acc)[MI][NI], const int lane,
+                                                      const int row_base, const int ncol_base, RowMap rowmap) {
+  static_assert(NI == 4, "a lane's four blocks are one 16-column group");
+  const int lm = lane & 15, lg = lane >> 4;
+  const float alpha = p.alpha;
+  const bool masked = (p.flags & L2S_F_MASK) != 0;
+  const int n0 = ncol_base + 16 * lg;
+  const bool ok_lo = n0 + 8 <= p.N, ok_hi = n0 + 16 <= p.N;
+  f32x4_t bj[NI];
+#pragma unroll
+  for (int j = 0; j < NI; ++j) {
+    bj[j] = f32x4_t{0.f, 0.f, 0.f, 0.f};
+    if (p.bias && n0 + 4 * j + 4 <= p.N) {
+      const float4 q = *reinterpret_cast<const float4*>(p.bias + n0 + 4 * j);
+      bj[j] = f32x4_t{q.x, q.y, q.z, q.w};
+    }
+  }
+  constexpr int CHK = MI < 4 ? MI : 4;
+  auto do_chunk = [&](auto c0_tag) {
+    constexpr int c0 = decltype(c0_tag)::value;
+    int orow[CHK];
+    bool keep[CHK];
+#pragma unroll
+    for (int i = 0; i < CHK; ++i) {
+      orow[i] = (int)rowmap(row_base + (c0 + i) * 16 + lm);
+      keep[i] = true;
+      if (masked) {
+        const int os = orow[i] < 0 ? 0 : orow[i];
+        const int clip = (int)((unsigned)os / (unsigned)p.mask_T);
+        keep[i] = (os - clip * p.mask_T) < p.lens[clip] * p.mask_mul;
+      }
+    }
+#pragma unroll
+    for (int i = 0; i < CHK; ++i) {
+      float u[8];
+#pragma unroll
+      for (int j = 0; j < NI; ++j) {
+        f32x4_t v = acc[c0 + i][j] + bj[j];
+        if (alpha != 1.f) v = v * alpha;
+#pragma unroll
+        for (int q = 0; q < 2; ++q) u[2 * j + q] = keep[i] ? v[2 * q] * __builtin_amdgcn_rcpf(1.0f + __expf(-v[2 * q + 1])) : 0.f;
+      }
+      if (orow[i] >= 0 && ok_lo) {
+        uint16_t* q = (uint16_t*)p.C + (int64_t)orow[i] * p.ldc + (n0 >> 1);
+        if (ok_hi) *reinterpret_cast<uint4*>(q) = make_uint4(ET::pack2(u[0], u[1]), ET::pack2(u[2], u[3]), ET::pack2(u[4], u[5]), ET::pack2(u[6], u[7]));
+        else *reinterpret_cast<uint2*>(q) = make_uint2(ET::pack2(u[0], u[1]), ET::pack2(u[2], u[3]));
+      }
+    }
+  };
+  do_chunk(std::integral_constant<int, 0>{});
+  if constexpr (MI > CHK) do_chunk(std::integral_constant<int, CHK>{});
+  if constexpr (MI > 2 * CHK) do_chunk(std::integral_constant<int, 2 * CHK>{});
+  if constexpr (MI > 3 * CHK) do_chunk(std::integral_constant<int, 3 * CHK>{});
+  static_assert(MI <= 4 * CHK, "chunk list");
+}
+
 __device__ __forceinline__ f32x4_t dpp_row_ror8(f32x4_t v) {
   float r0, r1, r2, r3;
   asm volatile("s_nop 1\n\tv_mov_b32_dpp %0, %4 row_ror:8 row_mask:0xf bank_mask:0xf\n\t"
@@ -903,6 +967,7 @@
                                          RowMap rowmap) {
   if constexpr (EPI < L2S_EPI_G16A)
     epilogue_fast16<ET, MI, NI, (EPI - L2S_EPI_F16) / 2, ((EPI - L2S_EPI_F16) & 1) != 0>(p, acc, scr, lane, row_base, ncol_base, grp, rowmap);
+  else if constexpr (EPI == L2S_EPI_GLU) epilogue_impl<ET, MI, NI, L2S_F_MASK, true, false, true>(p, acc, scr, lane, row_base, ncol_base, grp, rowmap);
   else if constexpr (EPI == L2S_EPI_G16A) epilogue_impl<ET, MI, NI, F_G16A, true>(p, acc, scr, lane, row_base, ncol_base, grp, rowmap);
   else if constexpr (EPI == L2S_EPI_G16B) epilogue_impl<ET, MI, NI, F_G16B, true>(p, acc, scr, lane, row_base, ncol_base, grp, rowmap);
   else if constexpr (EPI == L2S_EPI_S32) {
diff --git a/lip2speech_unit_amd/csrc/tapgemm_f32.hip b/lip2speech_unit_amd/csrc/tapgemm_f32.hip
--- a/lip2speech_unit_amd/csrc/tapgemm_f32.hip
+++ b/lip2speech_unit_amd/csrc/tapgemm_f32.hip
@@ -170,6 +170,7 @@
 int l2s_tapgemm_f32_launch(const l2s_gemm_desc& d, hipStream_t st) {
   if (d.ktab) return L2S_EUNSUPPORTED;
   if (d.mode < 0 || d.mode > 2) return L2S_EINVAL;
+  if (d.act == L2S_ACT_GLU) return L2S_EUNSUPPORTED;
   if ((d.Cin & 3) || (d.lda & 3) || (d.a_gstride & 3) || (d.w_gstride & 3)) return L2S_EALIGN;
   const int64_t tiles_m = ((int64_t)d.M + BM - 1) / BM, tiles_n = (d.N + BN - 1) / BN;
   if (tiles_m * tiles_n >= ((int64_t)1 << 31) || d.groups > 65535) return L2S_EUNSUPPORTED;
diff --git a/lip2speech_unit_amd/csrc/tapgemm_tiles.h b/lip2speech_unit_amd/csrc/tapgemm_tiles.h
--- a/lip2speech_unit_amd/csrc/tapgemm_tiles.h
+++ b/lip2speech_unit_amd/csrc/tapgemm_tiles.h
@@ -27,13 +27,15 @@
        L2S_EPI_S32 = 8,
        L2S_EPI_ALL = 9,
        L2S_EPI_COUNT = 10,
-       L2S_EPI_X32 = 10 };
+       L2S_EPI_X32 = 10,
+       L2S_EPI_GLU = 11 };
 inline bool is_x32(int flags, int act) {
   const int need = 0x2  | 0x20 , may = 0x4  | 0x8  | 0x10 ;
   return act == 0 && (flags & need) == need && (flags & ~(need | may)) == 0;
 }
 inline int pick_epilogue(int flags, int act) {
   const bool lin = act == 0  || act == 1  || act == 4  || act == 5 ;
+  if (act == 7 ) return L2S_EPI_GLU;
   if ((flags & ~0x10) == 0) {
     const int m = (flags & 0x10) ? 1 : 0;
     if (act == 0) return L2S_EPI_F16 + 0 + m;
diff --git a/lip2speech_unit_amd/ops.py b/lip2speech_unit_amd/ops.py
--- a/lip2speech_unit_amd/ops.py
+++ b/lip2speech_unit_amd/ops.py
@@ -5,7 +5,7 @@
 import torch
 
 from . import _lib
-from ._lib import (ACT_GELU, ACT_LRELU, ACT_NONE, ACT_PRELU, ACT_RELU, ACT_SWISH, ACT_TANH, BF16, F16, F32, F_ACCUM,
+from ._lib import (ACT_GELU, ACT_GLU, ACT_LRELU, ACT_NONE, ACT_PRELU, ACT_RELU, ACT_SWISH, ACT_TANH, BF16, F16, F32, F_ACCUM,
                    F_DUAL, F_MASK, F_OUT_F32, F_RES_F32, F_RES_POST, F_RES_PRE, MODE_CONV1D, MODE_CONV2D,
                    MODE_LINEAR, GemmDesc, L2SError, check)
 
@@ -108,7 +108,7 @@
         raise L2SError("lens must be int32")
     d.M, d.N, d.Cin, d.ntaps = M, N, Cin, ntaps
     d.lda = lda if lda is not None else Cin
-    d.ldc = ldc if ldc is not None else N * groups
+    d.ldc = ldc if ldc is not None else (N // 2 if act == ACT_GLU else N * groups)
     d.ldc2 = ldc2 if ldc2 is not None else d.ldc
     d.ldr = ldr if ldr is not None else d.ldc
     d.mode = mode
@@ -143,7 +143,7 @@
     osz = 4 if dtype == F32 else 2
     esz = 4 if (flags & F_OUT_F32) else osz
     mn = float(M) * N * groups
-    nbytes = float(osz) * M * ktot * groups / max(ntaps, 1) + float(osz) * N * ktot * groups + esz * mn
+    nbytes = float(osz) * M * ktot * groups / max(ntaps, 1) + float(osz) * N * ktot * groups + esz * mn * (0.5 if act == ACT_GLU else 1.0)
     if R is not None:
         nbytes += (4 if (flags & F_RES_F32) else osz) * mn
     if flags & F_DUAL:
@@ -206,6 +206,12 @@
 def glu_dwconv_swish(x, w, bias, y, *, B, T, C, k, lens=None, len_mul=1, dtype=F16):
     _run("l2s_glu_dwconv_swish", lambda: _lib.load().l2s_glu_dwconv_swish(_ptr(x), _ptr(w), _ptr(bias), _ptr(y), _ptr(lens), len_mul, B, T, C, k,
                                            dtype, _stream()))
+
+
+def dwconv_swish(u, w, bias, y, *, B, T, C, k, lens=None, len_mul=1, dtype=F16, max_blocks=0):
+    _run("l2s_dwconv_swish", lambda: _lib.load().l2s_dwconv_swish(_ptr(u), _ptr(w), _ptr(bias), _ptr(y), _ptr(lens), len_mul, B, T, C, k,
+                                                                dtype, max_blocks, _stream()),
+         flops=2.0 * B * T * C * k, nbytes=4.0 * B * T * C)
 
 
 def greedy_decode(logits, tokens, lprobs, score, *, B, T2, V, ldl=None, lens=None, len_mul=1, temperature=1.0,
@@ -772,6 +778,7 @@
     "layernorm": _LN,
     "attention": _ATT,
     "glu_dwconv_swish": _GLU,
+    "dwconv_swish": _GLU[:-7] + ", int max_blocks=0) -> ()",
     "greedy_decode": _GD,
     "beam_decode": "(Tensor logits, *, int B, int T2, int V, int beam, int? ldl=None, Tensor? lens=None, int len_mul=1, "
                    "float temperature=1.0, float lenpen=1.0) -> (Tensor, Tensor, Tensor, Tensor)",
```

Result: no change. 13490 (-0.1%).
